# skitzoid/Box2D-MT

Measured on AMD Instinct MI355X. Metric: world steps/sec at 99858 bodies per GPU (BASELINE config 3: Tumbler 100k, CCD off; Step = collide + island solve + broad-phase + state read-back); for N > 1: container-steps/s = world steps/s x N containers in the one sharded world, higher is better.
Workload: dtype f32

## Files before the change

### box2d-mt_amd/csrc/b2d_kernels_collide.h

```cpp
#ifndef B2D_KERNELS_COLLIDE_H
#define B2D_KERNELS_COLLIDE_H

#include "b2d_world.h"
#include "b2d_toi.h"

__device__ __forceinline__ Xf loadXf(const float4* b_xf, int body)
{
	float4 t = b_xf[body];
	Xf xf;
	xf.p = v2(t.x, t.y);
	xf.q.s = t.z;
	xf.q.c = t.w;
	return xf;
}

__device__ __forceinline__ AABB loadAabb(const float4* p_fat, int proxy)
{
	float4 t = p_fat[proxy];
	AABB a;
	a.lo = v2(t.x, t.y);
	a.hi = v2(t.z, t.w);
	return a;
}

__device__ __forceinline__ bool bodyActiveForContact(uint32_t f)
{
	return (f & BF_AWAKE) != 0 && (f & BF_TYPE_MASK) != BT_STATIC;
}

__device__ __forceinline__ bool filterShouldCollide(uint32_t f0A, int f1A, uint32_t f0B, int f1B)
{
	int groupA = (int)(short)(f1A & 0xffff);
	int groupB = (int)(short)(f1B & 0xffff);
	if (groupA == groupB && groupA != 0)
	{
		return groupA > 0;
	}
	uint32_t catA = f0A & 0xffffu, maskA = f0A >> 16;
	uint32_t catB = f0B & 0xffffu, maskB = f0B >> 16;
	return (maskA & catB) != 0 && (catA & maskB) != 0;
}

__device__ __forceinline__ bool bodiesShouldCollide(const DW& W, int bodyA, int bodyB)
{
	uint32_t tA = W.b_flags[bodyA] & BF_TYPE_MASK;
	uint32_t tB = W.b_flags[bodyB] & BF_TYPE_MASK;
	if (tA != BT_DYNAMIC && tB != BT_DYNAMIC) return false;
	if (W.nJoints == 0) return true;
	for (int e = W.jadjStart[bodyA], end = W.jadjStart[bodyA + 1]; e < end; ++e)
	{
		const JointRec& jn = W.joints[W.jadj[e]];
		if (jn.bodyA == bodyB || jn.bodyB == bodyB)
		{
			if (jn.collideConnected == 0) return false;
		}
	}
	return true;
}

__device__ __forceinline__ bool isToiCandidate(const DW& W, int proxyA, int proxyB, int bodyA, int bodyB)
{
	const int fA = W.p_filter1[proxyA], fB = W.p_filter1[proxyB];
	if ((fA | fB) & PF_SENSOR) return false;
	const uint32_t bfA = W.b_flags[bodyA], bfB = W.b_flags[bodyB];
	if ((bfA | bfB) & BF_BULLET) return true;
	const bool includesNonDynamic = (bfA & BF_TYPE_MASK) != BT_DYNAMIC || (bfB & BF_TYPE_MASK) != BT_DYNAMIC;
	const bool neitherThick = ((fA | fB) & PF_THICK) == 0;
	return includesNonDynamic && neitherThick;
}

#define TOI_ORDER_SORT_MAX 2048
#define TOI_ORDER_SCRATCH_BYTES (TOI_ORDER_SORT_MAX * (8 + 4 * 4))
__device__ __forceinline__ void toiOrderDestroy(const DW& W, void* scratch)
{
	DState* S = W.st;
	const int n = __hip_atomic_load(&S->c.nToiDestroy, __ATOMIC_RELAXED, __HIP_MEMORY_SCOPE_AGENT);
	if (n == 0) return;
	const ContactArrays& C = W.ca[S->cur];
	uint64_t* s_key = (uint64_t*)scratch;
	int* s_sorted = (int*)(s_key + TOI_ORDER_SORT_MAX);
	int* s_slot = s_sorted + TOI_ORDER_SORT_MAX;
	int* s_tail = s_slot + TOI_ORDER_SORT_MAX;
	int* s_tailJ = s_tail + TOI_ORDER_SORT_MAX;
	const bool chunked = n > TOI_ORDER_SORT_MAX;
	uint64_t* g_key = W.pairKey;
	int* g_sorted = (int*)(W.pairKey + n);
	int* g_rank = W.toiList;
// ... 36 lines not shown
				for (int j = 0; j < m; ++j) rank += s_key[j] < key ? 1 : 0;
				const int ci = b2dLoadAgentI(&W.toiDestroyList[i]);
				s_sorted[rank] = ci;
				s_slot[rank] = C.mgr[ci];
			}
		}
		else
		{
			for (int i = threadIdx.x; i < m; i += blockDim.x)
			{
				const int ci = g_sorted[c0 + i];
				s_sorted[i] = ci;
				s_slot[i] = b2dLoadAgentI(&C.mgr[ci]);
			}
		}
		for (int t = threadIdx.x; t < count0 - base; t += blockDim.x) s_tail[t] = b2dLoadAgentI(&W.toiPos2c[base + t]);
		__syncthreads();
		for (int t = threadIdx.x; t < count0 - base; t += blockDim.x)
		{
			const int c = s_tail[t];
			int j = -1;
			if (b2dLoadAgentI((const int*)&C.flags[c]) & (int)CF_DESTROY)
			{
				if (!chunked) { for (int q = 0; q < m; ++q) if (s_sorted[q] == c) { j = q; break; } }
				else { const int r = g_rank[c]; if (r >= c0 && r < c0 + m) j = r - c0; }
			}
			s_tailJ[t] = j;
		}
		__syncthreads();
		if (threadIdx.x == 0)
		{
			for (int k = 0; k < m; ++k)
			{
				const int ci = s_sorted[k];
				const int slot = s_slot[k];
				--count;
				const int last = s_tail[count - base], lastJ = s_tailJ[count - base];
				W.toiPos2c[slot] = last;
				C.mgr[last] = slot;
				if (slot >= base) { s_tail[slot - base] = last; s_tailJ[slot - base] = lastJ; }
				if (lastJ >= 0) s_slot[lastJ] = slot;
				C.mgr[ci] = -1;
			}
			__threadfence();
		}
		count = count0 - m;
		__syncthreads();
	}
	if (threadIdx.x == 0)
	{
		S->c.nToiOrder = count;
		S->c.nToiDestroy = 0;
	}
}

__device__ __forceinline__ int collideClassKey(const DW& W, const ContactArrays& C, int i)
{
	const int4 ids = C.ids[i];
	const uint32_t flags = C.flags[i];
	if (flags & CF_FOREIGN) return 61;
	if (!(bodyActiveForContact(W.b_flags[ids.z]) || bodyActiveForContact(W.b_flags[ids.w]))) return 62;
	const float4 fA = W.p_fat[ids.x], fB = W.p_fat[ids.y];
	if (fB.x - fA.z > 0.0f || fB.y - fA.w > 0.0f || fA.x - fB.z > 0.0f || fA.y - fB.w > 0.0f) return 62;
	if (flags & CF_SENSOR) return 60;
	const ShapeRec* sA = W.shapes + W.p_shape[ids.x];
	const ShapeRec* sB = W.shapes + W.p_shape[ids.y];
	const int tA = sA->type == B2D_SHAPE_CHAIN ? B2D_SHAPE_EDGE : sA->type, tB = sB->type;
	const int cA = sA->count, cB = sB->count;
	auto bucket = [](int c) { return c < 3 ? 0 : (c > 8 ? 5 : c - 3); };
	if (tA == B2D_SHAPE_POLYGON && tB == B2D_SHAPE_POLYGON) return bucket(cA > cB ? cA : cB);
	if (tA == B2D_SHAPE_POLYGON && tB == B2D_SHAPE_CIRCLE) return 6 + bucket(cA);
	if (tA == B2D_SHAPE_CIRCLE && tB == B2D_SHAPE_CIRCLE) return 12;
	if (tA == B2D_SHAPE_EDGE && tB == B2D_SHAPE_POLYGON) return 13 + bucket(cB);
	if (tA == B2D_SHAPE_EDGE && tB == B2D_SHAPE_CIRCLE) return 19;
	return 59;
}

__device__ __forceinline__ bool b2dSameBits4(float4 a, float4 b)
{
	return __float_as_uint(a.x) == __float_as_uint(b.x) && __float_as_uint(a.y) == __float_as_uint(b.y) &&
		__float_as_uint(a.z) == __float_as_uint(b.z) && __float_as_uint(a.w) == __float_as_uint(b.w);
}

template <int STAGE, bool ORDER = true>
__global__ __launch_bounds__(256) void
__attribute__((amdgpu_waves_per_eu((!ORDER && !STAGE) ? 4 : 1, (!ORDER && !STAGE) ? 4 : 8)))
k_collide(DW W, int sortTile)
{
	b2dPhaseStamp(W);
	DState* S = W.st;
	const int n = S->c.nContacts;
	const ContactArrays& C = W.ca[S->cur];
	int nDestroy = 0, nTouch = 0;
	__shared__ int s_bin[64];
	__shared__ int s_perm[256];
	__shared__ __attribute__((aligned(16))) unsigned char s_raw[STAGE ? ((512 * sizeof(ShapeRec) > TOI_ORDER_SCRATCH_BYTES || !ORDER) ? 512 * sizeof(ShapeRec) : TOI_ORDER_SCRATCH_BYTES) : (ORDER ? TOI_ORDER_SCRATCH_BYTES : 16)];
	ShapeRec* const s_shape = (ShapeRec*)s_raw;
	__shared__ __attribute__((aligned(16))) ShapeRec s_uni[2];
	__shared__ int s_uniId[2];
	const bool uniOn = !STAGE && (sortTile & 4) != 0;
	sortTile &= 3;
	if (uniOn)
	{
		const int i0 = (int)(blockIdx.x * blockDim.x);
		int idA = 0, idB = 0;
		if (i0 < n)
		{
			const int4 ids0 = C.ids[i0];
			idA = W.p_shape[ids0.x];
			idB = W.p_shape[ids0.y];
		}
		static_assert(sizeof(ShapeRec) % 4 == 0, "ShapeRec is copied word by word");
		constexpr int RW = (int)(sizeof(ShapeRec) / 4);
		if (threadIdx.x < 2 * RW)
		{
			const int which = (int)threadIdx.x / RW, word = (int)threadIdx.x % RW;
			((uint32_t*)&s_uni[which])[word] = ((const uint32_t*)(W.shapes + (which ? idB : idA)))[word];
		}
		if (threadIdx.x == 0) { s_uniId[0] = idA; s_uniId[1] = idB; }
		__syncthreads();
	}
	for (int base = blockIdx.x * blockDim.x; base < n; base += gridDim.x * blockDim.x)
	{
		int i = base + (int)threadIdx.x;
		if (sortTile)
		{
			const int key = i < n ? collideClassKey(W, C, i) : 63;
			if (threadIdx.x < 64) s_bin[threadIdx.x] = 0;
			__syncthreads();
			const int within = atomicAdd(&s_bin[key], 1);
			__syncthreads();
			if (threadIdx.x < 64)
			{
				const int v = s_bin[threadIdx.x];
				int incl = v;
				for (int off = 1; off < 64; off <<= 1)
				{
					const int o = __shfl_up(incl, off);
					if ((int)threadIdx.x >= off) incl += o;
				}
				s_bin[threadIdx.x] = incl - v;
			}
			__syncthreads();
			s_perm[s_bin[key] + within] = (int)threadIdx.x;
			__syncthreads();
			i = base + s_perm[threadIdx.x];
		}
		if (i >= n) continue;
		int4 ids = C.ids[i];
		uint32_t flags = C.flags[i];
		if (flags & CF_FOREIGN)
		{
			int keepF = 1;
			if (flags & CF_FILTER)
			{
				const bool ok = bodiesShouldCollide(W, ids.w, ids.z) &&
					filterShouldCollide(W.p_filter0[ids.x], W.p_filter1[ids.x], W.p_filter0[ids.y], W.p_filter1[ids.y]);
				if (!ok) keepF = 0; else flags &= ~CF_FILTER;
			}
			if (keepF && (bodyActiveForContact(W.b_flags[ids.z]) || bodyActiveForContact(W.b_flags[ids.w])))
			{
				const float4 fA = W.p_fat[ids.x], fB = W.p_fat[ids.y];
				AABB boxA, boxB;
				boxA.lo = v2(fA.x, fA.y); boxA.hi = v2(fA.z, fA.w);
				boxB.lo = v2(fB.x, fB.y); boxB.hi = v2(fB.z, fB.w);
				if (!b2dAabbOverlap(boxA, boxB)) keepF = 0;
			}
			if (!keepF)
			{
				flags |= CF_DESTROY;
				++nDestroy;
				if (flags & CF_TOI_CANDIDATE) b2dStoreAgentI(&W.toiDestroyList[atomicAdd(&S->c.nToiDestroy, 1)], i);
			}
			C.flags[i] = flags;
			W.keepFlag[i] = keepF;
			continue;
		}
		const int4 m3 = C.man3[i];
		const float4 oldImp = C.imp[i];
		const float4 o0 = C.man0[i], o1 = C.man1[i];
		const int proxyA = ids.x, proxyB = ids.y, bodyA = ids.z, bodyB = ids.w;
		uint32_t bfA = W.b_flags[bodyA], bfB = W.b_flags[bodyB];
		const float4 fatA = W.p_fat[proxyA], fatB = W.p_fat[proxyB];
		const int shapeA = W.p_shape[proxyA], shapeB = W.p_shape[proxyB];
		const Xf xfA = loadXf(W.b_xf, bodyA), xfB = loadXf(W.b_xf, bodyB);
		int keep = 1;

		if (flags & CF_FILTER)
		{
			bool ok = bodiesShouldCollide(W, bodyB, bodyA) &&
				(W.userFilter ? (flags & CF_USER_REJECT) == 0
				              : filterShouldCollide(W.p_filter0[proxyA], W.p_filter1[proxyA], W.p_filter0[proxyB], W.p_filter1[proxyB]));
			flags &= ~CF_USER_REJECT;
			if (!ok)
			{
				keep = 0;
			}
			else
			{
				flags &= ~CF_FILTER;
			}
		}

		flags &= ~(CF_PRESOLVE | CF_VC_ONE_POINT);
		bool active = bodyActiveForContact(bfA) || bodyActiveForContact(bfB);
		if (keep && active)
		{
			AABB boxA, boxB;
			boxA.lo = v2(fatA.x, fatA.y); boxA.hi = v2(fatA.z, fatA.w);
			boxB.lo = v2(fatB.x, fatB.y); boxB.hi = v2(fatB.z, fatB.w);
			bool overlap = b2dAabbOverlap(boxA, boxB);
			if (!overlap)
			{
				keep = 0;
			}
			else if (flags & CF_FOREIGN)
			{
			}
			else
			{
				const uint32_t oldId0 = (uint32_t)m3.x, oldId1 = (uint32_t)m3.y;
				const int oldCount = m3.w;
				flags |= CF_ENABLED;
				bool wasTouching = (flags & CF_TOUCHING) != 0;
				bool touching = false;
				bool sensor = (flags & CF_SENSOR) != 0;
				float4 o0s = make_float4(0, 0, 0, 0), o1s = o0s;
				Manifold mf;
				mf.pointCount = 0;
				mf.type = m3.z;
				mf.id[0] = oldId0;
				mf.id[1] = oldId1;
				if (sensor)
				{
					const GjkProxy pA = b2dProxy(W.shapes + shapeA);
					const GjkProxy pB = b2dProxy(W.shapes + shapeB);
					GjkCache cache;
					cache.count = 0;
					cache.metric = 0.0f;
					for (int k = 0; k < 3; ++k) cache.indexA[k] = cache.indexB[k] = 0;
					GjkOutput dist;
					b2dDistance(dist, cache, pA, xfA, pB, xfB, true);
					touching = dist.distance < 10.0f * B2D_EPSILON;
					mf.pointCount = 0;
				}
				else
				{
					const ShapeRec* sA = W.shapes + shapeA;
					const ShapeRec* sB = W.shapes + shapeB;
					if (STAGE)
					{
						static_assert(sizeof(ShapeRec) % 8 == 0, "ShapeRec is copied in 8-byte pieces");
						const float2* gA = (const float2*)sA;
						const float2* gB = (const float2*)sB;
						float2* lA = (float2*)&s_shape[2 * threadIdx.x];
						float2* lB = (float2*)&s_shape[2 * threadIdx.x + 1];
#pragma unroll
						for (int q = 0; q < (int)(sizeof(ShapeRec) / 8); ++q) { lA[q] = gA[q]; lB[q] = gB[q]; }
						sA = &s_shape[2 * threadIdx.x];
						sB = &s_shape[2 * threadIdx.x + 1];
					}
					o0s = o0;
					o1s = o1;
					mf.localNormal = v2(o0.x, o0.y);
					mf.localPoint = v2(o0.z, o0.w);
					mf.p[0] = v2(o1.x, o1.y);
					mf.p[1] = v2(o1.z, o1.w);
					mf.id[0] = oldId0;
					mf.id[1] = oldId1;
					bool evaluated = false;
					if (uniOn)
					{
						const int u0 = s_uniId[0], u1 = s_uniId[1];
						const bool a0 = shapeA == u0, b0 = shapeB == u0;
						if ((a0 || shapeA == u1) && (b0 || shapeB == u1))
						{
							const ShapeRec* lA = &s_uni[a0 ? 0 : 1];
							const ShapeRec* lB = &s_uni[b0 ? 0 : 1];
							if (lA->type == B2D_SHAPE_POLYGON && lB->type == B2D_SHAPE_POLYGON && lA->count == 4 && lB->count == 4)
							{
								b2dCollidePolygons<4>(&mf, lA, xfA, lB, xfB);
								evaluated = true;
							}
						}
					}
					if (!evaluated) b2dEvaluate(&mf, sA, xfA, sB, xfB);
					touching = mf.pointCount > 0;
					float ni[2], ti[2];
					ni[0] = oldImp.x; ti[0] = oldImp.y; ni[1] = oldImp.z; ti[1] = oldImp.w;
					for (int k = 0; k < mf.pointCount; ++k)
					{
						mf.ni[k] = 0.0f;
						mf.ti[k] = 0.0f;
						uint32_t id2 = mf.id[k];
						if (oldCount > 0 && oldId0 == id2)
						{
							mf.ni[k] = oldImp.x;
							mf.ti[k] = oldImp.y;
						}
						else if (oldCount > 1 && oldId1 == id2)
						{
							mf.ni[k] = oldImp.z;
							mf.ti[k] = oldImp.w;
						}
						ni[k] = mf.ni[k];
						ti[k] = mf.ti[k];
					}
					if (touching != wasTouching)
					{
						W.b_wake[bodyA] = 1;
					}
					{
						const float4 n0 = make_float4(mf.localNormal.x, mf.localNormal.y, mf.localPoint.x, mf.localPoint.y);
						const float4 n1 = make_float4(mf.p[0].x, mf.p[0].y, mf.p[1].x, mf.p[1].y);
						const float4 nI = make_float4(ni[0], ti[0], ni[1], ti[1]);
						if (!b2dSameBits4(n0, o0)) C.man0[i] = n0;
						if (!b2dSameBits4(n1, o1)) C.man1[i] = n1;
						if (!b2dSameBits4(nI, oldImp)) C.imp[i] = nI;
					}
				}
				if (W.preSolveOn && !sensor && touching)
				{
					W.pre_o0[i] = o0s;
					W.pre_o1[i] = o1s;
					W.pre_oimp[i] = oldImp;
					W.pre_o3[i] = m3;
					flags |= CF_PRESOLVE;
				}
				{
					const int4 n3 = make_int4((int)mf.id[0], (int)mf.id[1], mf.type, mf.pointCount);
					if (n3.x != m3.x || n3.y != m3.y || n3.z != m3.z || n3.w != m3.w) C.man3[i] = n3;
				}
				if (touching) flags |= CF_TOUCHING; else flags &= ~CF_TOUCHING;
			}
		}

		if (!keep)
		{
			if (W.eventsOn && (flags & CF_REPORTED))
			{
				const int e = atomicAdd(&S->c.nEvents, 1);
				if (e < W.capContacts)
				{
					W.evKey[e] = C.key[i];
					W.evInfo[e] = make_int4(proxyA, proxyB, 1, -1);
				}
			}
			flags |= CF_DESTROY;
			++nDestroy;
			if (flags & CF_TOI_CANDIDATE) b2dStoreAgentI(&W.toiDestroyList[atomicAdd(&S->c.nToiDestroy, 1)], i);
			int pc = C.man3[i].w;
			if (pc > 0 && (flags & (CF_SENSOR | CF_FOREIGN)) == 0)
			{
				W.b_wake[bodyA] = 1;
				W.b_wake[bodyB] = 1;
			}
		}
		else if ((flags & (CF_TOUCHING | CF_FOREIGN)) == CF_TOUCHING)
		{
			++nTouch;
		}
		C.flags[i] = flags;
		W.keepFlag[i] = keep;
	}
	{
		__shared__ int s_census[2];
		if (threadIdx.x == 0) { s_census[0] = 0; s_census[1] = 0; }
		__syncthreads();
		nDestroy = waveSumInt(nDestroy);
		nTouch = waveSumInt(nTouch);
		if (waveLane() == 0)
		{
			if (nDestroy) atomicAdd(&s_census[0], nDestroy);
			if (nTouch) atomicAdd(&s_census[1], nTouch);
		}
		__syncthreads();
		const bool fit = (unsigned)W.capContacts <= TREE_SUM_MAX;
		if (!fit && threadIdx.x == 0)
		{
			if (s_census[0]) atomicAdd(&S->c.nDestroy, s_census[0]);
			if (s_census[1]) atomicAdd(&S->c.nTouching, s_census[1]);
		}
		unsigned t0 = 0u, t1 = 0u;
		if (b2dLastBlockArrive(W, ARRIVE_COLLIDE, fit ? (unsigned)s_census[0] : 0u, fit ? (unsigned)s_census[1] : 0u, &t0, &t1))
		{
			if (threadIdx.x == 0)
			{
				if (t0) atomicAdd(&S->c.nDestroy, (int)t0);
				if (t1) atomicAdd(&S->c.nTouching, (int)t1);
			}
			if (ORDER) toiOrderDestroy(W, s_raw);
		}
	}
}

__global__ __launch_bounds__(256) void k_toi_order_destroy(DW W)
{
	__shared__ __attribute__((aligned(16))) unsigned char s_raw[TOI_ORDER_SCRATCH_BYTES];
	toiOrderDestroy(W, s_raw);
}

__global__ __launch_bounds__(256) void k_contact_events(DW W)
{
	b2dPhaseStamp(W);
	DState* S = W.st;
	const int n = S->c.nContacts;
	const ContactArrays& C = W.ca[S->cur];
	for (int i = blockIdx.x * blockDim.x + threadIdx.x; i < n; i += gridDim.x * blockDim.x)
	{
		const uint32_t flags = C.flags[i];
		const bool touching = (flags & CF_TOUCHING) != 0, reported = (flags & CF_REPORTED) != 0;
		if (touching == reported || (flags & CF_FOREIGN) != 0) continue;
		C.flags[i] = flags ^ CF_REPORTED;
		const int e = atomicAdd(&S->c.nEvents, 1);
		if (e < W.capContacts)
		{
			const int4 ids = C.ids[i];
			W.evKey[e] = C.key[i];
			W.evInfo[e] = make_int4(ids.x, ids.y, touching ? 0 : 1, i);
		}
	}
}

__global__ __launch_bounds__(256) void k_presolve_gather(DW W)
{
	b2dPhaseStamp(W);
	DState* S = W.st;
	const int n = S->c.nContacts;
	const bool compacting = S->c.nDestroy != 0;
	const ContactArrays& C = W.ca[S->cur];
	for (int i = blockIdx.x * blockDim.x + threadIdx.x; i < n; i += gridDim.x * blockDim.x)
	{
		if (!W.keepFlag[i] || (C.flags[i] & CF_PRESOLVE) == 0) continue;
		C.flags[i] &= ~CF_PRESOLVE_OFF;
		const int e = atomicAdd(&S->c.nPreSolve, 1);
		if (e >= W.capContacts) continue;
		const int4 ids = C.ids[i];
		PreSolveRec r;
		r.info = make_int4(compacting ? W.keepScan[i] : i, ids.x, ids.y, 0);
		r.key = C.key[i];
		r.pad = 0ull;
		r.o0 = W.pre_o0[i]; r.o1 = W.pre_o1[i]; r.oimp = W.pre_oimp[i]; r.o3 = W.pre_o3[i];
		r.n0 = C.man0[i]; r.n1 = C.man1[i]; r.nimp = C.imp[i]; r.n3 = C.man3[i];
		r.mat = C.mat[i];
		W.preRecs[e] = r;
	}
}

__global__ __launch_bounds__(256) void k_presolve_disable(DW W, const int* list, int count)
{
	b2dPhaseStamp(W);
	const ContactArrays& C = W.ca[W.st->cur];
	for (int k = blockIdx.x * blockDim.x + threadIdx.x; k < count; k += gridDim.x * blockDim.x)
	{
		const int j = list[k];
		if (j >= 0 && j < W.st->c.nContacts) C.flags[j] = (C.flags[j] & ~CF_ENABLED) | CF_PRESOLVE_OFF;
	}
}

__global__ __launch_bounds__(256) void k_presolve_material(DW W, const int* list, int count)
{
	b2dPhaseStamp(W);
	const ContactArrays& C = W.ca[W.st->cur];
	for (int k = blockIdx.x * blockDim.x + threadIdx.x; k < count; k += gridDim.x * blockDim.x)
	{
		const int j = list[4 * k];
		if (j < 0 || j >= W.st->c.nContacts) continue;
		float4 m = C.mat[j];
		m.x = __int_as_float(list[4 * k + 1]);
		m.y = __int_as_float(list[4 * k + 2]);
		m.z = __int_as_float(list[4 * k + 3]);
		C.mat[j] = m;
	}
}

__global__ __launch_bounds__(256) void k_postsolve_gather(DW W)
// ... 47 lines not shown
	}
}

__global__ __launch_bounds__(256) void k_pairs_reject(DW W, const int* list, int count)
{
	b2dPhaseStamp(W);
	for (int k = blockIdx.x * blockDim.x + threadIdx.x; k < count; k += gridDim.x * blockDim.x) W.pairFirst[list[k]] = 0;
}

__global__ void k_step_begin(DW W, int* bar)
{
	b2dPhaseStamp(W);
	Counters& c = W.st->c;
	const int t = threadIdx.x;
	if (t == 0)
	{
		c.nDestroy = 0;
		(&c.nDestroy)[1] = 0;
		c.nPairs = 0;
		(&c.nPairs)[1] = 0;
		c.overflow = 0;
		c.cellExtBits = 0;
		c.gridFresh = 0;
		W.st->dbgCensus[0] = 0;
		c.nEvents = 0;
		c.nToiList = 0;
		c.nNewToiCand = 0;
		c.nToiEvents = 0;
		c.nToiCalls = 0;
		c.toiBase = 0;
		c.toiOverflow = 0;
		c.nToiLog = 0;
		c.toiIncomplete = 0;
		c.toiUnsafe = 0;
		c.nToiGroups = 0;
		c.nToiMoved = 0;
		c.nToiNewPairs = 0;
		c.nToiChainCreated = 0;
		c.nPreSolve = 0;
		c.nPostSolve = 0;
		c.nFilterList = 0;
		c.spToiCreated = 0;
		c.spToiStraddle = 0;
	}
	if (t < 32) bar[t] = t == 6 ? W.testSpinMax : 0;
	for (int k = t; k < ARRIVE_SITES * TREE_WORDS; k += (int)blockDim.x) W.arriveTree[k] = 0ull;
}

__global__ __launch_bounds__(256) void k_wake_apply(DW W)
{
	b2dPhaseStamp(W);
	for (int i = blockIdx.x * blockDim.x + threadIdx.x; i < W.nBodies; i += gridDim.x * blockDim.x)
	{
		if (W.b_wake[i])
		{
			W.b_flags[i] |= BF_AWAKE;
			W.b_pos[i].w = 0.0f;
			W.b_wake[i] = 0;
		}
	}
}

__global__ __launch_bounds__(256) void k_flag_filter(DW W, const unsigned long long* pairs, int nPairs)
{
	b2dPhaseStamp(W);
	DState* S = W.st;
	const int n = S->c.nContacts;
	const ContactArrays& C = W.ca[S->cur];
	for (int i = blockIdx.x * blockDim.x + threadIdx.x; i < n; i += gridDim.x * blockDim.x)
	{
		const int4 ids = C.ids[i];
		const unsigned lo = (unsigned)(ids.z < ids.w ? ids.z : ids.w), hi = (unsigned)(ids.z < ids.w ? ids.w : ids.z);
		const unsigned long long key = ((unsigned long long)lo << 32) | hi;
		int a = 0, b = nPairs;
		while (a < b)
		{
			const int m = (a + b) >> 1;
			if (pairs[m] < key) a = m + 1; else b = m;
		}
		if (a < nPairs && pairs[a] == key) C.flags[i] |= CF_FILTER;
	}
}

struct DW;
__device__ __forceinline__ bool keysetMaintained(const DW& W);
__device__ __forceinline__ bool htDelete(const DW& W, uint32_t mask, uint64_t key);

__global__ __launch_bounds__(256) void k_compact_contacts(DW W)
{
	b2dPhaseStamp(W);
	DState* S = W.st;
	if (S->c.nDestroy == 0) return;
	const int n = S->c.nContacts;
	const ContactArrays& A = W.ca[S->cur];
	const ContactArrays& B = W.ca[1 - S->cur];
	const bool ksOn = keysetMaintained(W);
	const uint32_t ksMask = S->c.ksMask;
	int ksTomb = 0, ksLost = 0;
	__shared__ int s_ks[2];
	if (threadIdx.x == 0) { s_ks[0] = 0; s_ks[1] = 0; }
	__syncthreads();
	for (int i = blockIdx.x * blockDim.x + threadIdx.x; i < n; i += gridDim.x * blockDim.x)
	{
		const int keep = W.keepFlag[i];
		const uint32_t fl = A.flags[i];
		const uint64_t key = A.key[i];
		if (!keep)
		{
			if (ksOn && (fl & CF_FOREIGN) == 0)
			{
				if (htDelete(W, ksMask, key + 1ull)) ksTomb += 1;
				else ksLost += 1;
			}
		}
		else
		{
			int j = W.keepScan[i];
			B.ids[j] = A.ids[i];
			B.key[j] = key;
			B.flags[j] = fl;
			if ((fl & CF_FOREIGN) == 0)
			{
				B.mat[j] = A.mat[i];
				B.man0[j] = A.man0[i];
				B.man1[j] = A.man1[i];
				B.imp[j] = A.imp[i];
				B.man3[j] = A.man3[i];
			}
			B.color[j] = A.color[i];
			const int m = A.mgr[i];
			B.mgr[j] = m;
			if (m >= 0) W.toiPos2c[m] = j;
		}
	}
	const bool fit = (unsigned)W.capContacts <= TREE_SUM_MAX;
	if (ksOn)
	{
		ksTomb = waveSumInt(ksTomb);
		ksLost = waveSumInt(ksLost);
		if (waveLane() == 0)
		{
			if (ksTomb) atomicAdd(&s_ks[0], ksTomb);
			if (ksLost) atomicAdd(&s_ks[1], ksLost);
		}
	}
	__syncthreads();
	unsigned tomb = (unsigned)s_ks[0], lost = (unsigned)s_ks[1];
	if (!fit && threadIdx.x == 0)
	{
		if (tomb) atomicAdd(&S->c.ksStats[KS_TOMBSTONES], (unsigned long long)tomb);
		if (lost) { atomicAdd(&S->c.ksStats[KS_NOT_FOUND], (unsigned long long)lost); S->c.ksStale = 1; }
	}
	if (b2dLastBlockArrive(W, ARRIVE_COMPACT, fit ? tomb : 0u, fit ? lost : 0u, &tomb, &lost) && threadIdx.x == 0)
	{
		if (fit && tomb) S->c.ksStats[KS_TOMBSTONES] += (unsigned long long)tomb;
		if (fit && lost) { S->c.ksStats[KS_NOT_FOUND] += (unsigned long long)lost; S->c.ksStale = 1; }
		S->c.nContacts = W.keepScan[n];
		S->cur = 1 - S->cur;
	}
}

#define HT_TOMB 0xffffffffffffffffull

__device__ __forceinline__ uint32_t hashKey(uint64_t k)
{
	k ^= k >> 33;
	k *= 0xff51afd7ed558ccdULL;
	k ^= k >> 33;
	k *= 0xc4ceb9fe1a85ec53ULL;
	k ^= k >> 33;
// ... 99 lines not shown
```

### box2d-mt_amd/csrc/b2hip_api_callbacks.h

```cpp

int b2hip_set_contact_filter(b2hip_world* w, b2hip_should_collide_fn fn, void* user)
{
	if (int rcu = checkUsable(w, "b2hip_set_contact_filter", true)) return rcu;
	w->filterFn = fn;
	w->filterUser = user;
	w->dw.userFilter = hasFilter(w) ? 1 : 0;
	return B2HIP_OK;
}

int b2hip_set_contact_filter_batch(b2hip_world* w, b2hip_should_collide_batch_fn fn, void* user)
{
	if (int rcu = checkUsable(w, "b2hip_set_contact_filter_batch", true)) return rcu;
	w->filterBatchFn = fn;
	if (fn) w->filterUser = user;
	w->dw.userFilter = hasFilter(w) ? 1 : 0;
	return B2HIP_OK;
}

int b2hip_default_should_collide(b2hip_world* w, int fixture_a, int fixture_b)
{
	if (!w || fixture_a < 0 || fixture_b < 0 || fixture_a >= (int)w->fixtures.size() || fixture_b >= (int)w->fixtures.size())
		return setError(B2HIP_ERR_INVALID, "bad fixture id");
	const HostFixture& a = w->fixtures[fixture_a];
	const HostFixture& b = w->fixtures[fixture_b];
// ... 121 lines not shown
		std::vector<uint32_t> f(nb);
		if (nb && hipMemcpy(f.data(), w->b_flags.p, nb * 4, hipMemcpyDeviceToHost) != hipSuccess) bad = 1;
		for (size_t i = 0; i < nb; ++i) f[i] &= 0x7fu;
		h = fnv(h, f.data(), nb * 4);
	}
	else if (which == 1)
	{
		bad |= pull(w->c_ids[cur].p, nc * 16); bad |= pull(w->c_key[cur].p, nc * 8);
		std::vector<uint32_t> f(nc);
		if (nc && hipMemcpy(f.data(), w->c_flags[cur].p, nc * 4, hipMemcpyDeviceToHost) != hipSuccess) bad = 1;
		for (size_t i = 0; i < nc; ++i) f[i] &= 0x1fu;
		h = fnv(h, f.data(), nc * 4);
		bad |= pull(w->c_man0[cur].p, nc * 16); bad |= pull(w->c_man1[cur].p, nc * 16);
		bad |= pull(w->c_imp[cur].p, nc * 16); bad |= pull(w->c_man3[cur].p, nc * 16);
	}
	else if (which == 2)
	{
		bad |= pull(w->p_fat.p, np * 16);
	}
	else
	{
		bad |= pull(w->c_imp[cur].p, nc * 16);
	}
	if (bad) return setError(B2HIP_ERR_HIP, "debug hash read-back failed");
	*out = h;
	return 0;
}

int b2hip_debug_read(b2hip_world* w, int which, int first, int count, void* out)
{
	if (!w) return setError(B2HIP_ERR_INVALID, "null world");
	DEVICE_GUARD(w);
	if (!w || !out) return setError(B2HIP_ERR_INVALID, "null argument");
	HIP_TRY(hipStreamSynchronize(w->stream));
	const void* src = nullptr;
	size_t elem = 16;
	switch (which)
	{
	case 0: src = w->b_pos.p; break;
	case 1: src = w->b_vel.p; break;
	case 2: src = w->li_bodies.p; elem = 4; break;
	case 3: src = w->b_force.p; break;
	case 4: src = w->b_flags.p; elem = 4; break;
	case 5: src = w->b_damp.p; break;
	case 6: src = w->b_mass.p; break;
	case 7: src = w->d_state.p; elem = 4; break;
	case 8: src = w->dbgPreVel.p; break;
	case 9: src = w->dbgVel.p; break;
	case 10: src = w->dbgLi.p; elem = 4; break;
	case 11: src = w->gridBar.p; elem = 4; break;
	case 12:
	{
		if (first < 0 || count < 0 || first + count > COLOR_SLOT_PADDED) return setError(B2HIP_ERR_INVALID, "colour census: [0, 65)");
		HIP_TRY(hipStreamSynchronize(w->stream));
		if (count > 0) HIP_TRY(hipMemcpy2D(out, sizeof(int), w->colorCount.p + colorSlot(first), COLOR_SLOT_STRIDE * sizeof(int), sizeof(int), (size_t)count, hipMemcpyDeviceToHost));
		return 0;
	}
	case 13: src = w->bodyColorMask.p; elem = 8; break;
	case 14: src = w->deg.p; elem = 4; break;
	case 15: src = w->hubList.p; elem = 4; break;
	case 16: src = w->bodyActive.p; elem = 8; break;
	case 17: src = w->b_blk1.p; elem = 4; break;
	case 18: src = w->li_ref.p; break;
	case 19: src = w->rowColor.p; elem = 4; break;
	case 20: src = w->blkRowStart.p; elem = 4; break;
	case 21: src = w->bodyRest.p; elem = 8; break;
	case 22:
	{
		const long long stats[2] = { w->statSorts, w->statSortsOnepass };
		if (first < 0 || count < 0 || first + count > 2) return setError(B2HIP_ERR_INVALID, "pair-update statistics: [0, 2)");
		memcpy(out, stats + first, (size_t)count * sizeof(long long));
		return 0;
	}
	case 23:
	{
		if (first < 0 || count < 0 || first + count > KS_STATS + 2) return setError(B2HIP_ERR_INVALID, "key-set statistics: [0, 12)");
		Counters c;
		HIP_TRY(hipMemcpy(&c, &w->d_state.p->c, sizeof(Counters), hipMemcpyDeviceToHost));
		long long stats[KS_STATS + 2];
		for (int k = 0; k < KS_STATS; ++k) stats[k] = (long long)c.ksStats[k];
		stats[KS_STATS] = c.ksFill;
		stats[KS_STATS + 1] = c.ksMask;
		memcpy(out, stats + first, (size_t)count * sizeof(long long));
		return 0;
	}
	default: return setError(B2HIP_ERR_INVALID, "bad array id");
	}
	HIP_TRY(hipMemcpy(out, (const char*)src + (size_t)first * elem, (size_t)count * elem, hipMemcpyDeviceToHost));
	return 0;
}

int b2hip_test_radix_sort(b2hip_world* w, int count, uint64_t* keys, int* payloads, int passes, const int* shifts, const int* widths)
{
	if (!w) return setError(B2HIP_ERR_INVALID, "null world");
	DEVICE_GUARD(w);
	if (count < 0 || passes < 1 || !shifts || !widths || (count > 0 && (!keys || !payloads))) return setError(B2HIP_ERR_INVALID, "bad argument");
	if (w->stepActive) return setError(B2HIP_ERR_INVALID, "inside a step");
	std::vector<std::pair<int, int>> lay;
	for (int p = 0; p < passes; ++p)
	{
		if (widths[p] < 1 || widths[p] > RADIX_BITS || shifts[p] < 0 || shifts[p] + widths[p] > 64) return setError(B2HIP_ERR_INVALID, "bad pass");
		lay.push_back(std::make_pair(shifts[p], widths[p]));
	}
	int rc = ensureCapacity(w, 0);
	if (rc) return rc;
	hipStream_t s = w->stream;
	const int tilesCap = count / RADIX_TILE + 1;
	const size_t tiles = (size_t)tilesCap + 1;
	rc = w->radixHist.ensure(RADIX_DIGITS * tiles + 2, s); if (rc) return rc;
	rc = w->radixHistScan.ensure(RADIX_DIGITS * tiles + 4, s); if (rc) return rc;
	rc = w->scanTmp.ensure(3 * (RADIX_DIGITS * tiles / SCAN_TILE + 8), s); if (rc) return rc;
	rc = w->scanFlags.ensure(RADIX_DIGITS * tiles / SCAN_TILE + 8, s); if (rc) return rc;
	if (w->sortOnepass)
	{
		const size_t onepassTiles = std::min<size_t>(tiles, RADIX_ONEPASS_MAX_TILES);
		rc = w->radixCounts.ensure(onepassTiles * RADIX_DIGITS, s, false); if (rc) return rc;
		rc = w->radixGroups.ensure((onepassTiles / RADIX_GROUP + 1) * RADIX_DIGITS, s, false); if (rc) return rc;
	}
	rc = ensureCapacity(w, 0);
	if (rc) return rc;
	DevArray<uint64_t> k0, k1;
	DevArray<int2> v0, v1;
	DevArray<int> nDev;
	const size_t room = (size_t)count + 1;
	rc = k0.ensure(room, s, false, false);
	if (!rc) rc = k1.ensure(room, s, false, false);
	if (!rc) rc = v0.ensure(room, s, false, false);
	if (!rc) rc = v1.ensure(room, s, false, false);
	if (!rc) rc = nDev.ensure(1, s, false, true);
	auto done = [&](int code) { (void)hipStreamSynchronize(s); k0.release(); k1.release(); v0.release(); v1.release(); nDev.release(); return code; };
	if (rc) return done(rc);
	hipError_t e = hipMemcpyAsync(nDev.p, &count, sizeof(int), hipMemcpyHostToDevice, s);
	if (e == hipSuccess && count > 0) e = hipMemcpyAsync(k0.p, keys, (size_t)count * sizeof(uint64_t), hipMemcpyHostToDevice, s);
	if (e == hipSuccess && count > 0) e = hipMemcpyAsync(v0.p, payloads, (size_t)count * sizeof(int2), hipMemcpyHostToDevice, s);
	if (e != hipSuccess) return done(setError(B2HIP_ERR_HIP, hipGetErrorString(e)));
	uint64_t *kin = k0.p, *kout = k1.p;
	int2 *vin = v0.p, *vout = v1.p;
	rc = radixSort(w, kin, kout, vin, vout, nDev.p, tilesCap, lay);
	if (rc) return done(rc);
	int overflow = 0;
	e = hipMemcpyAsync(&overflow, &w->d_state.p->c.overflow, sizeof(int), hipMemcpyDeviceToHost, s);
	if (e == hipSuccess && count > 0) e = hipMemcpyAsync(keys, kin, (size_t)count * sizeof(uint64_t), hipMemcpyDeviceToHost, s);
	if (e == hipSuccess && count > 0) e = hipMemcpyAsync(payloads, vin, (size_t)count * sizeof(int2), hipMemcpyDeviceToHost, s);
	if (e == hipSuccess) e = hipStreamSynchronize(s);
	if (e != hipSuccess) return done(setError(B2HIP_ERR_HIP, hipGetErrorString(e)));
	if (overflow & SCAN_ABORT_BIT) return done(setError(B2HIP_ERR_HIP, "a look-back of the sort gave up waiting for a predecessor tile"));
	return done(0);
}

__global__ __launch_bounds__(256) void k_keyset_check(DW W, unsigned long long* out)
{
	const DState* S = W.st;
	const ContactArrays& C = W.ca[S->cur];
	const uint32_t mask = S->c.ksMask;
	const int stride = (int)(gridDim.x * blockDim.x), t0 = (int)(blockIdx.x * blockDim.x + threadIdx.x);
	int missing = 0, own = 0, live = 0, tomb = 0;
	for (int i = t0; i < S->c.nContacts; i += stride)
	{
		if (C.flags[i] & CF_FOREIGN) continue;
		own += 1;
		const uint64_t key = C.key[i] + 1ull;
		uint32_t h = hashKey(key) & mask;
		bool found = false;
		for (uint32_t probes = 0; probes <= mask; ++probes)
		{
			const uint64_t v = W.ht_keys[h];
// ... 172 lines not shown
```

### box2d-mt_amd/csrc/b2hip_api_snapshot.h

```cpp

namespace
{
struct SnapHeader
{
	char magic[8];
	uint32_t version, szDState, szHostBody, szHostFixture, szShape, szJoint;
	uint32_t nBodies, nFixtures, nShapes, nJoints, nFree, nContacts, nToiOrder, nMoves;
	uint32_t stateCount, cur;
	int32_t nextNode, leafCount, lastContacts, newFixture;
	float inv_dt0, cellSize;
	int32_t eventsOn, solverHints;
};
const uint32_t kSnapVersion = 6;
const char kSnapMagic[8] = { 'B', '2', 'H', 'I', 'P', 'S', 'N', '1' };

struct SnapWriter
{
	std::vector<char> out;
	void host(const void* p, size_t n) { const char* c = (const char*)p; out.insert(out.end(), c, c + n); }
	int dev(const void* p, size_t n)
	{
		const size_t at = out.size();
		out.resize(at + n);
		if (n == 0) return 0;
// ... 197 lines not shown
	{
		uint32_t tail[2];
		in.host(tail, sizeof(tail));
		if (tail[1] != sizeof(GearRec) || tail[0] > size) return corrupt("gear section");
		nG = tail[0];
		gearsAt = (const GearRec*)in.take(nG * sizeof(GearRec));
		if (!gearsAt && nG) return setError(B2HIP_ERR_INVALID, "snapshot truncated");
	}
	for (size_t k = 0; k < nJ; ++k)
	{
		RevoluteJoint j;
		memcpy((void*)&j, jointsAt + k, sizeof(j));
		if (j.type < B2D_JOINT_DEAD || j.type > B2D_JOINT_GEAR) return corrupt("joint type");
		if (j.bodyA < 0 || (size_t)j.bodyA >= nb || j.bodyB < 0 || (size_t)j.bodyB >= nb) return corrupt("joint bodies");
		if (j.type == B2D_JOINT_GEAR && (j.enableLimit < 0 || (size_t)j.enableLimit >= nG)) return corrupt("gear index");
	}
	for (size_t k = 0; k < nG; ++k)
	{
		GearRec g;
		memcpy((void*)&g, gearsAt + k, sizeof(g));
		if (g.bodyC < 0 || (size_t)g.bodyC >= nb || g.bodyD < 0 || (size_t)g.bodyD >= nb) return corrupt("gear bodies");
	}

	def.device = device;
	b2hip_world* w = nullptr;
	int rc = b2hip_world_create(&def, &w);
	if (rc) return rc;
	DEVICE_GUARD(w);
	auto fail = [&](int code) { const std::string why = g_lastError; b2hip_world_destroy(w); return setError(code, why); };
	w->bodies.resize(nb);
	for (size_t i = 0; i < nb; ++i)
	{
		memcpy((void*)&w->bodies[i], bodiesAt + i * bodyBytes, offsetof(HostBody, fixtures));
		w->bodies[i].dirty = bodiesAt[i * bodyBytes + offsetof(HostBody, fixtures)] != 0;
		w->bodies[i].pullEpoch = 0;
		w->bodies[i].forceEpoch = w->stepEpoch;
		if (w->bodies[i].dirty) w->dirtyList.push_back((int)i);
	}
	{
		size_t count = 0;
		for (size_t i = 0; i < nb; ++i) count += w->bodies[i].worldIndex >= 0 ? 1 : 0;
		w->nonStatic.assign(count, -1);
		for (size_t i = 0; i < nb; ++i)
		{
			const int k = w->bodies[i].worldIndex;
			if (k < 0) continue;
			if ((size_t)k >= count || w->nonStatic[(size_t)k] != -1) return fail(corrupt("non-static body order"));
			w->nonStatic[(size_t)k] = (int)i;
		}
		w->orderDirty = true;
	}
	w->fixtures.resize(np);
	if (np) memcpy(w->fixtures.data(), fixturesAt, np * sizeof(HostFixture));
	w->shapes.resize(nS);
	if (nS) memcpy((void*)w->shapes.data(), shapesAt, nS * sizeof(ShapeRec));
	w->freeUnits.resize(h.nFree);
	if (h.nFree) memcpy(w->freeUnits.data(), freeAt, (size_t)h.nFree * sizeof(FreeUnit));
	for (size_t f = 0; f < np; ++f) w->bodies[w->fixtures[f].body].fixtures.push_back((int)f);
	for (size_t k = 0; k < nS; ++k) w->shapeIndex[std::string((const char*)&w->shapes[k], sizeof(ShapeRec))] = (int)k;
	w->joints.resize(nJ);
	if (nJ) memcpy((void*)w->joints.data(), jointsAt, nJ * sizeof(RevoluteJoint));
	for (size_t k = 0; k < nJ; ++k) w->nMouseJoints += w->joints[k].type == B2D_JOINT_MOUSE;
	w->gears.resize(nG);
	if (nG) memcpy((void*)w->gears.data(), gearsAt, nG * sizeof(GearRec));
	w->nextNode = h.nextNode; w->leafCount = h.leafCount; w->lastContacts = h.lastContacts; w->newFixture = h.newFixture != 0;
	w->inv_dt0 = h.inv_dt0;
	w->eventsOn = h.eventsOn != 0;
	w->serialOrphansNext = h.solverHints & 1;
	w->blocksTooBig = (h.solverHints & 2) != 0;
	w->stepComplete = (h.solverHints & 4) == 0;
	w->adoptSticky = (h.solverHints >> 8) & 0xff;
	w->largeHintSteps = (h.solverHints >> 16) & 0xff;
	w->recolorCountdown = (h.solverHints >> 24) & 0x7f;
	w->freshColors = ((h.solverHints >> 3) & 0x1f) | ((int)(((uint32_t)h.solverHints >> 31) & 1u) << 5);
	w->freshColorsPending = false;
	w->adoptPasses = w->adoptSticky > 0;
	rc = ensureCapacity(w, nC);
	if (rc) return fail(rc);
	if (nM > w->moveBuf.cap || nC > (size_t)w->dw.capContacts || (size_t)h.stateCount * 10 > w->h_stateCap) return fail(corrupt("counts exceed the buffers sized for them"));
	if (h.stateCount) memcpy(w->h_state, stateAt, (size_t)h.stateCount * 10 * sizeof(float));
	w->shadowDev = nullptr;
	w->stateCount = h.stateCount;
	*w->h_dstate = ds;
#define SNAP_UP(arr, s) do { if ((s).bytes && hipMemcpy(w->arr.p, (s).p, (s).bytes, hipMemcpyHostToDevice) != hipSuccess) return fail(setError(B2HIP_ERR_HIP, "snapshot upload failed (" #arr ")")); } while (0)
	if (hipMemcpy(w->d_state.p, &ds, sizeof(DState), hipMemcpyHostToDevice) != hipSuccess) return fail(setError(B2HIP_ERR_HIP, "snapshot upload failed (state block)"));
	w->pubSeq = ds.pubCount;
	SNAP_UP(b_pos, sPos); SNAP_UP(b_pos0, sPos0); SNAP_UP(b_vel, sVel); SNAP_UP(b_xf, sXf); SNAP_UP(b_mass, sMass); SNAP_UP(b_damp, sDamp);
	w->forceOnDevice = true; w->rowsWentEarly = false;
	SNAP_UP(b_force, sForce); SNAP_UP(b_flags, sFlags); SNAP_UP(b_wake, sWake); SNAP_UP(b_proxyHead, sHead); SNAP_UP(b_blk1, sBlk);
	SNAP_UP(p_fat, sFat); SNAP_UP(p_body, sPBody); SNAP_UP(p_shape, sPShape); SNAP_UP(p_key, sPKey); SNAP_UP(p_filter0, sF0); SNAP_UP(p_filter1, sF1);
	SNAP_UP(p_mat, sPMat); SNAP_UP(p_next, sNext);
	const int cur = (int)h.cur;
	SNAP_UP(c_ids[cur], cIds); SNAP_UP(c_key[cur], cKey); SNAP_UP(c_flags[cur], cFlags); SNAP_UP(c_mat[cur], cMat); SNAP_UP(c_man0[cur], cMan0);
	SNAP_UP(c_man1[cur], cMan1); SNAP_UP(c_imp[cur], cImp); SNAP_UP(c_man3[cur], cMan3); SNAP_UP(c_color[cur], cColor); SNAP_UP(c_mgr[cur], cMgr);
	SNAP_UP(toiPos2c, sToi); SNAP_UP(moveBuf, sMoves);
#undef SNAP_UP
	if (nS && hipMemcpy(w->d_shapes.p, w->shapes.data(), nS * sizeof(ShapeRec), hipMemcpyHostToDevice) != hipSuccess)
		return fail(setError(B2HIP_ERR_HIP, "snapshot upload failed (shapes)"));
	w->upBodies = nb; w->upFixtures = np; w->upShapes = nS; w->upJoints = 0;
	w->dw.cellSize = h.cellSize;
	w->dw.invCellSize = 1.0f / h.cellSize;
	w->dw.eventsOn = w->eventsOn ? 1 : 0;
	*out = w;
	return B2HIP_OK;
}

int b2hip_get_contacts(b2hip_world* w, int cap, b2hip_contact* out)
{
	if (!w) return setError(B2HIP_ERR_INVALID, "null world");
	DEVICE_GUARD(w);
	if (!w || !out) return setError(B2HIP_ERR_INVALID, "null argument");
	int rc = flushForRead(w);
	if (rc) return rc;
	rc = readState(w);
	if (rc) return rc;
	const int n = std::min(cap, w->h_dstate->c.nContacts);
	const int cur = w->h_dstate->cur;
	if (n <= 0) return 0;
	std::vector<int4> ids(n), m3(n);
	std::vector<uint32_t> flags(n);
	std::vector<float4> mat(n), m0(n), m1(n), imp(n);
	HIP_TRY(hipMemcpy(ids.data(), w->c_ids[cur].p, n * sizeof(int4), hipMemcpyDeviceToHost));
	HIP_TRY(hipMemcpy(m3.data(), w->c_man3[cur].p, n * sizeof(int4), hipMemcpyDeviceToHost));
	HIP_TRY(hipMemcpy(flags.data(), w->c_flags[cur].p, n * sizeof(uint32_t), hipMemcpyDeviceToHost));
	HIP_TRY(hipMemcpy(mat.data(), w->c_mat[cur].p, n * sizeof(float4), hipMemcpyDeviceToHost));
	HIP_TRY(hipMemcpy(m0.data(), w->c_man0[cur].p, n * sizeof(float4), hipMemcpyDeviceToHost));
	HIP_TRY(hipMemcpy(m1.data(), w->c_man1[cur].p, n * sizeof(float4), hipMemcpyDeviceToHost));
	HIP_TRY(hipMemcpy(imp.data(), w->c_imp[cur].p, n * sizeof(float4), hipMemcpyDeviceToHost));
	for (int i = 0; i < n; ++i)
	{
		b2hip_contact& c = out[i];
		c.fixture_a = ids[i].x;
		c.fixture_b = ids[i].y;
		c.body_a = ids[i].z;
		c.body_b = ids[i].w;
		c.flags = ((flags[i] & CF_TOUCHING) ? 1u : 0u) | ((flags[i] & CF_ENABLED) ? 2u : 0u);
		c.manifold_type = m3[i].z;
		c.point_count = m3[i].w;
		c.local_normal[0] = m0[i].x; c.local_normal[1] = m0[i].y;
		c.local_point[0] = m0[i].z; c.local_point[1] = m0[i].w;
		c.point_local[0][0] = m1[i].x; c.point_local[0][1] = m1[i].y;
		c.point_local[1][0] = m1[i].z; c.point_local[1][1] = m1[i].w;
		c.normal_impulse[0] = imp[i].x; c.tangent_impulse[0] = imp[i].y;
		c.normal_impulse[1] = imp[i].z; c.tangent_impulse[1] = imp[i].w;
		c.id_key[0] = (uint32_t)m3[i].x;
		c.id_key[1] = (uint32_t)m3[i].y;
		c.friction = mat[i].x;
		c.restitution = mat[i].y;
		c.tangent_speed = mat[i].z;
	}
	return n;
}
```

### box2d-mt_amd/csrc/b2hip_api_step.h

```cpp

int b2hip_step_begin(b2hip_world* w, float dt, int velocity_iterations, int position_iterations)
{
	if (int rc = checkUsable(w, "b2hip_step_begin", false)) return rc;
	if (w->stepActive) return setError(B2HIP_ERR_INVALID, "b2hip_step_begin inside a step (finish it with b2hip_step_end)");
	DEVICE_GUARD(w);
	return stepFailed(w, stepBeginImpl(w, dt, velocity_iterations, position_iterations));
}

static bool keyLess(const std::pair<unsigned long long, int>& a, const std::pair<unsigned long long, int>& b) { return a < b; }

static void toManifold(b2hip_manifold* m, float4 m0, float4 m1, float4 imp, int4 m3)
{
	m->type = m3.z;
	m->point_count = m3.w;
	m->local_normal[0] = m0.x; m->local_normal[1] = m0.y;
	m->local_point[0] = m0.z; m->local_point[1] = m0.w;
	m->point_local[0][0] = m1.x; m->point_local[0][1] = m1.y;
	m->point_local[1][0] = m1.z; m->point_local[1][1] = m1.w;
	m->normal_impulse[0] = imp.x; m->tangent_impulse[0] = imp.y;
	m->normal_impulse[1] = imp.z; m->tangent_impulse[1] = imp.w;
	m->id_key[0] = (uint32_t)m3.x;
	m->id_key[1] = (uint32_t)m3.y;
}

// ... 557 lines not shown
		}
	}
	w->events.clear();
	if (w->h_dstate->c.rowsSkipped == 1)
	{
		rc = downloadState(w, -1);
		if (rc) return rc;
	}
	if (w->eventsOn)
	{
		LAUNCH(w, k_contact_events, gridFor(w->dw.capContacts), 256, w->dw);
		int nEv = 0;
		HIP_TRY(hipMemcpyAsync(&nEv, &w->d_state.p->c.nEvents, sizeof(int), hipMemcpyDeviceToHost, w->stream));
		HIP_TRY(hipStreamSynchronize(w->stream));
		if (nEv > w->dw.capContacts) return setError(B2HIP_ERR_CAPACITY, "contact event buffer overflow");
		if (nEv > 0)
		{
			std::vector<unsigned long long> keys(nEv);
			std::vector<int4> info(nEv);
			HIP_TRY(hipMemcpy(keys.data(), w->evKey.p, nEv * sizeof(unsigned long long), hipMemcpyDeviceToHost));
			HIP_TRY(hipMemcpy(info.data(), w->evInfo.p, nEv * sizeof(int4), hipMemcpyDeviceToHost));
			std::vector<int> order(nEv);
			for (int i = 0; i < nEv; ++i) order[i] = i;
			std::sort(order.begin(), order.end(), [&](int a, int b)
			{
				if (info[a].z != info[b].z) return info[a].z < info[b].z;
				return keys[a] < keys[b];
			});
			w->events.resize(nEv);
			for (int i = 0; i < nEv; ++i)
			{
				const int4 q = info[order[i]];
				w->events[i].fixture_a = q.x;
				w->events[i].fixture_b = q.y;
				w->events[i].kind = q.z;
				w->events[i].contact_index = q.w;
			}
		}
	}
	if (w->debugSync) HIP_TRY(hipStreamSynchronize(w->stream));
	refreshMirror(w);
	const Counters& c = w->h_dstate->c;
	w->lastContacts = c.nContacts;
	w->last.nContacts = c.nContacts;
	w->last.nMoves = c.nMoves;
	if (c.nMovesSeen > 256 && !w->gridForced)
	{
		long long rounds = 0;
		for (int k = 0; k < 32; ++k) rounds += c.candRounds[k];
		const double perProxy = 64.0 * (double)rounds / (double)c.nMovesSeen;
		if (perProxy > 128.0) w->gridHalf = true; else if (perProxy < 48.0) w->gridHalf = false;
		w->dw.gridHalf = w->gridHalf ? 1 : 0;
	}
	w->last.nNewContacts = c.nNewContacts;
	w->last.nPairs = c.nPairs;
	w->last.overflow = c.overflow;
	if (w->colorSmallPending)
	{
		w->colorSmallPending = false;
		w->last.nColors = c.nColors;
		if (c.overflow & 4) return setError(B2HIP_ERR_CAPACITY, "more than 64 constraint colours on one body");
		if (c.nUncolored != 0) return setError(B2HIP_ERR_CAPACITY, "incremental colouring did not converge");
	}
	if ((c.overflow & 0x2040) == 0x2040) return setError(B2HIP_ERR_CAPACITY, "a block of the large-island partition holds more rows or home bodies than its workgroup takes (the census the host partitions by did not see them)");
	if (c.overflow & 64)
	{
		if (w->handoverWhy) handoverPostMortem(w);
		return setError(B2HIP_ERR_HIP, "a wait inside a resident large-island solver timed out (a workgroup was not resident, or a hand-over never came)");
	}
	if (c.overflow & SCAN_ABORT_BIT) return setError(B2HIP_ERR_HIP, "a single-pass scan gave up waiting for a predecessor tile (k_scan_chain look-back)");
	w->last.posItersLarge = c.posItersLarge;
	w->last.nHubRows = c.nHubRows;
	w->last.hubRounds = c.hubRounds;
	w->last.hubSerialChunks = c.hubSerialChunks;
	w->toiChainContacts += c.nToiChainCreated;
	if (w->toiRan)
	{
		w->last.toiUnsafe = c.toiUnsafe;
		w->last.nToiEvents = c.nToiEvents;
		w->last.nToiCalls = c.nToiCalls;
		w->last.toiOverflow = c.toiOverflow;
		if (c.toiOverflow) return setError(B2HIP_ERR_CAPACITY, "TOI event scratch overflow (flags " + std::to_string(c.toiOverflow) + ")");
	}
	if (w->sp.dt > 0.0f) w->inv_dt0 = w->sp.inv_dt;
	if (w->def.continuous && w->sp.dt > 0.0f) w->stepComplete = c.toiIncomplete == 0;
	w->stepActive = false;

	float ms = 0.0f;
	float* p = w->profile;
	memset(p, 0, sizeof(float) * 13);
	{
		const unsigned long long* pc0 = w->h_dstate->phaseClock;
		p[0] = pc0[13] > pc0[14] ? 1.0e-5f * (float)(pc0[13] - pc0[14]) : 0.0f;
	}
	if (w->profileDetail)
	{
	const unsigned long long* pc = w->h_dstate->phaseClock;
	auto span = [pc](int a, int b) -> float { return pc[b] > pc[a] ? 1.0e-5f * (float)(pc[b] - pc[a]) : 0.0f; };
	p[1] = span(1, 2);
	p[2] = span(2, 3);
	p[3] = span(2, 4);
	const float dfs = span(4, 5), small = span(5, 6), color = span(6, 7), large = span(7, 8);
	p[3] += dfs + color;
	p[5] = small + large;
	const float bpTop = span(0, 1), bp0 = span(3, 9), bp1 = span(9, 10);
	p[10] = bp0;
	p[11] = bp1 + bpTop;
	p[9] = bp0 + bp1 + bpTop;
	if (w->toiEventValid) p[7] = span(10, 12);
	w->solverMs = small + large;
	if (w->blocksThisStep && w->h_dstate->stamps[4] > 0)
	{
		const float tick = 1.0e-5f;
		const float total = tick * (float)w->h_dstate->stamps[4];
		const float scale = total > 0.0f ? large / total : 0.0f;
		p[4] = scale * tick * (float)w->h_dstate->stamps[0];
		p[5] = small + scale * tick * (float)(w->h_dstate->stamps[2] - w->h_dstate->stamps[0]);
		p[6] = scale * tick * (float)(w->h_dstate->stamps[4] - w->h_dstate->stamps[2]);
	}
	}
	const int Ct = w->last.nSContacts + w->last.nLContacts;
	const int B = w->last.nSBodies + w->last.nLBodies;
	w->solverConstraints = Ct;
	w->solverBodies = B;
	w->solverBytes = (double)Ct * (w->sp.velIters * 220.0 + w->sp.posIters * 136.0 + 488.0) + (double)B * 240.0;
	w->ktMs = 0.0f;
	w->ktLaunches = 0;
	w->ktBytes = 0.0;
	if (w->kernelTiming && w->ktUsed >= 2)
	{
		for (int k = 0; k + 1 < w->ktUsed; k += 2)
		{
			float t = 0.0f;
			(void)hipEventElapsedTime(&t, w->ktEvents[k], w->ktEvents[k + 1]);
			w->ktMs += t;
			w->ktLaunches += 1;
		}
		if (w->ktKind == 5) w->ktBytes = (double)w->ktUnitsA * 480.0 + (double)w->ktUnitsB * 230.0;
		else if (w->ktKind == 6) w->ktBytes = (double)w->ktUnitsA * 250.0;
		else if (w->ktKind == 7) w->ktBytes = (double)w->ktUnitsA * 16.0 + (double)w->ktUnitsB * 8.0;
		else if (w->ktKind == 1) w->ktBytes = (double)w->last.nLContacts * 220.0 * w->sp.velIters;
		else if (w->ktKind == 8)
		{
			w->ktBytes = (double)w->last.nLContacts * (w->sp.velIters * 220.0 + w->last.posItersLarge * 136.0 + 488.0) + (double)w->last.nLBodies * 240.0;
			w->ktLaunches = w->familyLaunches;
		}
		else if (w->ktKind == 4) w->ktBytes = (double)w->last.nLContacts * (w->sp.velIters * 220.0 + w->last.posItersLarge * 136.0 + 488.0) + (double)w->last.nLBodies * 240.0;
		else w->ktBytes = (double)w->last.nSContacts * (w->sp.velIters * 220.0 + w->sp.posIters * 136.0 + 488.0) + (double)w->last.nSBodies * 240.0;
	}
	return 0;
}

int b2hip_set_lazy_readback(b2hip_world* w, int enable)
{
	if (int rc = checkUsable(w, "b2hip_set_lazy_readback", true)) return rc;
	ensureRows(w);
	w->lazyReadback = enable != 0;
	return w->failed ? setError(B2HIP_ERR_HIP, w->failedWhy) : B2HIP_OK;
}

int b2hip_step_end(b2hip_world* w)
{
	if (int rc = checkUsable(w, "b2hip_step_end", false)) return rc;
	if (!w->stepActive) return setError(B2HIP_ERR_INVALID, "b2hip_step_end outside a step");
	DEVICE_GUARD(w);
	const int rc = stepFailed(w, stepEndImpl(w));
// ... 88 lines not shown
```

### box2d-mt_amd/csrc/b2hip_api_world.h

```cpp


const char* b2hip_last_error(void)
{
	return g_lastError.c_str();
}

const char* b2hip_version(void)
{
	return "b2hip 0.1 (gfx950)";
}

int b2hip_world_create(const b2hip_world_def* def, b2hip_world** out)
{
	if (!def || !out) return setError(B2HIP_ERR_INVALID, "null argument");
	int count = 0;
	hipError_t e = hipGetDeviceCount(&count);
	if (e != hipSuccess || count <= 0)
	{
		return setError(B2HIP_ERR_NO_DEVICE, "no HIP device available: the b2hip Step() path has no CPU fallback");
	}
	int current = 0;
	if (hipGetDevice(&current) != hipSuccess) current = 0;
	const int device = def->device >= 0 ? def->device : current;
	if (device >= count) return setError(B2HIP_ERR_NO_DEVICE, "no such HIP device");
// ... 102 lines not shown
		return setError(B2HIP_ERR_HIP, "hipHostMalloc failed");
	}
	if (hipHostMalloc((void**)&w->h_pub, sizeof(DState), hipHostMallocMapped | hipHostMallocCoherent) != hipSuccess ||
		hipHostGetDevicePointer((void**)&w->d_pub, w->h_pub, 0) != hipSuccess)
	{
		b2hip_world_destroy(w);
		return setError(B2HIP_ERR_HIP, "hipHostMalloc (coherent) failed");
	}
	memset(w->h_pub, 0, sizeof(DState));
	if (hipHostMalloc((void**)&w->h_pub2, sizeof(DState), hipHostMallocMapped | hipHostMallocCoherent) != hipSuccess ||
		hipHostGetDevicePointer((void**)&w->d_pub2, w->h_pub2, 0) != hipSuccess)
	{
		b2hip_world_destroy(w);
		return setError(B2HIP_ERR_HIP, "hipHostMalloc (coherent) failed");
	}
	memset(w->h_pub2, 0, sizeof(DState));
	if (hipHostMalloc((void**)&w->h_solverWord, 64, hipHostMallocMapped | hipHostMallocCoherent) != hipSuccess ||
		hipHostGetDevicePointer((void**)&w->d_solverWord, w->h_solverWord, 0) != hipSuccess)
	{
		b2hip_world_destroy(w);
		return setError(B2HIP_ERR_HIP, "hipHostMalloc (coherent) failed");
	}
	memset(w->h_solverWord, 0, 64);
	int rc = ensureCapacity(w, 0);
	if (rc == 0 && hipStreamSynchronize(w->stream) != hipSuccess) rc = setError(B2HIP_ERR_HIP, "stream sync failed");
	if (rc)
	{
		const std::string why = g_lastError;
		b2hip_world_destroy(w);
		return setError(rc, why);
	}
	*out = w;
	return B2HIP_OK;
}

void b2hip_world_destroy(b2hip_world* w)
{
	if (!w) return;
	DEVICE_GUARD(w);
	if (w->stream) (void)hipStreamSynchronize(w->stream);
	if (w->rowStream)
	{
		(void)hipStreamSynchronize(w->rowStream);
		(void)hipStreamDestroy(w->rowStream);
		(void)hipEventDestroy(w->rowFork);
		(void)hipEventDestroy(w->rowJoin);
		w->rowStream = nullptr;
	}
	if (w->shardComm != nullptr && g_rcclDestroy != nullptr) g_rcclDestroy(w->shardComm);
	w->shardComm = nullptr;
	w->shardSend.release(); w->shardRecv.release();
	w->b_owner.release(); w->spNewOwner.release(); w->spAwake.release(); w->spStraddle.release(); w->spCount.release(); w->spTarget.release();
	w->spSend.release(); w->spRecv.release(); w->spTailKey.release(); w->spVirt.release();
	if (w->spHost) (void)hipHostFree(w->spHost);
	w->spHost = nullptr;
	if (w->spOwnHost) (void)hipHostFree(w->spOwnHost);
	w->spOwnHost = nullptr;
	if (w->spHdrHost) (void)hipHostFree(w->spHdrHost);
	w->spHdrHost = nullptr;
	for (size_t k = 0; k < w->spTape.size(); ++k) (void)hipFree(w->spTape[k].first);
	w->spTape.clear();
	w->d_state.release();
	w->b_pos.release(); w->b_pos0.release(); w->b_vel.release(); w->b_xf.release(); w->b_mass.release(); w->b_damp.release();
	w->b_force.release(); w->b_flags.release(); w->b_wake.release(); w->b_rowDirty.release();
	w->p_fat.release(); w->p_body.release(); w->p_shape.release(); w->p_key.release(); w->p_filter0.release(); w->p_filter1.release();
	w->p_mat.release(); w->d_shapes.release();
	for (int k = 0; k < 2; ++k)
	{
		w->c_ids[k].release(); w->c_key[k].release(); w->c_flags[k].release(); w->c_mat[k].release(); w->c_man0[k].release();
		w->c_man1[k].release(); w->c_imp[k].release(); w->c_man3[k].release(); w->c_color[k].release();
	}
	w->ht_keys.release(); w->d_joints.release(); w->d_gears.release(); w->li_ref.release();
	w->jadjStart.release(); w->jadj.release(); w->rootJointStart.release(); w->rootJointCursor.release();
	w->lj_list.release(); w->rootJointOkay.release();
	w->parent.release(); w->rootSeed.release(); w->rootBodies.release(); w->rootContacts.release(); w->rootJoints.release();
	w->rootIsland.release(); w->deg.release(); w->adjStart.release(); w->adjCursor.release(); w->adj.release(); w->adjSlot.release();
	w->rootScanIn.release(); w->rootScanOut.release();
	w->si_root.release(); w->si_bodyStart.release(); w->si_contactStart.release(); w->si_wStart.release(); w->si_maxLevel.release();
	w->si_bodies.release(); w->si_contacts.release(); w->si_level.release(); w->si_stack.release(); w->si_lastLevel.release();
	w->b_slot.release(); w->b_island.release(); w->chunkFirst.release();
	w->li_bodies.release(); w->li_contacts.release(); w->li_roots.release(); w->li_color.release(); w->colorCount.release();
	w->colorStart.release(); w->colorCursor.release(); w->li_sorted.release(); w->bodyClaim.release(); w->rootPen.release();
	w->bodyActive.release(); w->bodyRest.release(); w->b_posv.release(); w->evKey.release(); w->evInfo.release(); w->uncolList.release(); w->compactList.release(); w->gridBar.release(); w->hubRowOf.release(); w->hubList.release(); w->hubDelta.release(); w->hubMeta.release(); w->hubFirst.release(); w->solveSnapBody.release(); w->solveSnapImp.release(); w->solveSnapCFlags.release(); w->solveSnapJoints.release(); w->solveSnapGears.release();
	w->b_proxyHead.release(); w->p_next.release(); w->toiList.release(); w->toiPos2c.release(); w->toiDestroyList.release(); w->toiNewList.release();
	w->b_toiGroup.release(); w->toiGroups.release(); w->toiGroupCount.release(); w->toiGroupList.release(); w->toiMoved.release(); w->toiNew.release(); w->toiParent.release(); w->toiDomOf.release(); w->toiDomRoot.release(); w->toiDomCount.release(); w->toiDomBase.release(); w->toiDomFill.release(); w->toiDomFailed.release(); w->toiDomEvents.release(); w->toiDomList.release(); w->toiHull.release(); w->snapBody.release(); w->snapFat.release();
	w->c_mgr[0].release(); w->c_mgr[1].release(); w->dbgPreVel.release(); w->dbgVel.release(); w->dbgLi.release();
	w->rootSleepMin.release(); w->bodyColorMask.release(); w->rootDone.release(); w->lc.release(); w->warmDelta.release();
	w->moveBuf.release(); w->gridCount.release(); w->gridStart.release(); w->gridCursor.release(); w->gridItems.release(); w->gridFat.release(); w->arriveTree.release();
	w->largeProxies.release(); w->largeMoves.release(); w->pairKey.release(); w->pairKey2.release(); w->pairProxy.release(); w->pairProxy2.release();
	w->filterPairs.release();
	w->d_editOps.release();
	w->b_order.release(); w->orderBody.release(); w->bigRoots.release();
	w->pre_o0.release(); w->pre_o1.release(); w->pre_oimp.release(); w->pre_o3.release(); w->preRecs.release();
	w->postRecs.release(); w->filterList.release(); w->hostList.release(); w->toiLog.release(); w->toiVerdict.release();
	w->b_blk1.release(); w->b_adopt.release(); w->b_adoptStage.release(); w->blkRows.release(); w->blkRowStart.release(); w->blkCursor.release(); w->blkBodyCount.release(); w->blkBodyCursor.release();
	w->blkBodyStart.release(); w->blkBodies.release(); w->rowColor.release(); w->b_cutv.release();
	w->pairFirst.release(); w->pairRank.release(); w->scanTmp.release(); w->radixHist.release(); w->radixHistScan.release();
	w->keepFlag.release(); w->keepScan.release(); w->scanTmp4.release(); w->scanFlags.release(); w->radixCounts.release(); w->radixGroups.release(); w->radixGlobalHist.release(); w->stateOut.release(); w->consts.release();
	w->qIn.release(); w->qCounts.release(); w->qOffsets.release(); w->qItems.release(); w->qFlags.release(); w->qScanWork.release();
	w->qScanWords.release(); w->qWords.release(); w->qHits.release(); w->qDistances.release(); w->qPoses.release(); w->qShapes.release();
	w->qKeys.release(); w->qKeysWork.release(); w->qAny.release();
	if (w->qPinned) (void)hipHostFree(w->qPinned);
	if (w->h_state) (void)hipHostFree(w->h_state);
	if (w->h_dstate) (void)hipHostFree(w->h_dstate);
	if (w->h_pub) (void)hipHostFree(w->h_pub);
	if (w->h_pub2) (void)hipHostFree(w->h_pub2);
	if (w->h_solverWord) (void)hipHostFree(w->h_solverWord);
	for (int i = 0; i < 13; ++i)
		if (w->ev[i]) (void)hipEventDestroy(w->ev[i]);
	for (size_t i = 0; i < w->ktEvents.size(); ++i) (void)hipEventDestroy(w->ktEvents[i]);
	if (w->stream) (void)hipStreamDestroy(w->stream);
	if (w->stream2) (void)hipStreamDestroy(w->stream2);
	if (w->evFork) (void)hipEventDestroy(w->evFork);
	if (w->evJoin) (void)hipEventDestroy(w->evJoin);
	delete w;
}

int b2hip_set_gravity(b2hip_world* w, float gx, float gy)
{
	if (int rcu = checkUsable(w, "b2hip_set_gravity", true)) return rcu;
	if (!w) return setError(B2HIP_ERR_INVALID, "null world");
	w->def.gravity_x = gx;
	w->def.gravity_y = gy;
	return 0;
}

int b2hip_set_flags(b2hip_world* w, int allow_sleep, int warm_starting, int continuous, int sub_stepping)
{
	if (int rcu = checkUsable(w, "b2hip_set_flags", true)) return rcu;
	if (!w) return setError(B2HIP_ERR_INVALID, "null world");
	w->def.allow_sleep = allow_sleep;
	w->def.warm_starting = warm_starting;
	w->def.continuous = continuous;
	w->def.sub_stepping = sub_stepping;
	return 0;
}

int b2hip_create_body(b2hip_world* w, const b2hip_body_def* def)
{
	if (!w || !def) return setError(B2HIP_ERR_INVALID, "null argument");
	if (int rcu = checkUsable(w, "b2hip_create_body", true)) return rcu;
	HostBody b{};
	b.type = def->type;
	b.flags = 0;
	if (def->bullet) b.flags |= BF_BULLET;
	if (def->fixed_rotation) b.flags |= BF_FIXEDROT;
	if (def->allow_sleep) b.flags |= BF_AUTOSLEEP;
	if (def->awake) b.flags |= BF_AWAKE;
	if (def->active) b.flags |= BF_ACTIVE;
	b.px = def->px;
	b.py = def->py;
	b.qs = sinf(def->angle);
	b.qc = cosf(def->angle);
	b.lcx = b.lcy = 0.0f;
	b.c0x = b.cx = def->px;
	b.c0y = b.cy = def->py;
	b.a0 = b.a = def->angle;
	b.vx = def->vx;
	b.vy = def->vy;
	b.w = def->w;
	b.linearDamping = def->linear_damping;
	b.angularDamping = def->angular_damping;
	b.gravityScale = def->gravity_scale;
	b.fx = b.fy = b.torque = 0.0f;
	b.sleepTime = 0.0f;
	b.pullEpoch = w->mirrorEpoch;
	b.forceEpoch = w->stepEpoch;
// ... 1121 lines not shown
```

### box2d-mt_amd/csrc/b2hip_host_phases.h

```cpp

static int spExchangeState(b2hip_world* w, int mode);
static int spExchangePairs(b2hip_world* w, long long* totalPairs, int* straddling);
static int spResolve(b2hip_world* w, int nVirt = 0);
static int spAfterToi(b2hip_world* w);
static int spBeginStep(b2hip_world* w);

static int radixBits(int maxKey)
{
	int bits = 1;
	while ((1 << bits) <= maxKey && bits < 31) ++bits;
	return bits;
}

static void radixPasses(int first, int bits, std::vector<std::pair<int, int>>& out)
{
	const int passes = (bits + RADIX_BITS - 1) / RADIX_BITS;
	for (int p = 0, at = 0; p < passes; ++p)
	{
		const int width = (bits - at + (passes - p) - 1) / (passes - p);
		out.push_back(std::make_pair(first + at, width));
		at += width;
	}
}

// ... 66 lines not shown

static int userFilterPairs(b2hip_world* w, const int2* proxies)
{
	int rc = readState(w);
	if (rc) return rc;
	const int n = std::min(w->h_dstate->c.nPairs, w->dw.capPairs);
	if (n <= 0 || (w->h_dstate->c.overflow & 3)) return 0;
	std::vector<int> first(n);
	std::vector<int2> pr(n);
	HIP_TRY(hipMemcpy(first.data(), w->pairFirst.p, (size_t)n * sizeof(int), hipMemcpyDeviceToHost));
	HIP_TRY(hipMemcpy(pr.data(), proxies, (size_t)n * sizeof(int2), hipMemcpyDeviceToHost));
	std::vector<int> refused, asked, which, verdict;
	for (int i = 0; i < n; ++i)
	{
		if (!first[i]) continue;
		asked.push_back(pr[i].x);
		asked.push_back(pr[i].y);
		which.push_back(i);
	}
	askFilter(w, asked, verdict);
	for (size_t k = 0; k < which.size(); ++k) if (!verdict[k]) refused.push_back(which[k]);
	return applyHostList(w, k_pairs_reject, refused);
}

static int runSortAndCreate(b2hip_world* w, bool largePath, long long knownPairs = -1)
{
	DW& d = w->dw;
	const uint64_t* sortedKeys = d.pairKey;
	const int2* sortedProxies = d.pairProxy;
	if (largePath)
	{
		int bits = radixBits(w->nextNode + 1);
		std::vector<std::pair<int, int>> passes;
		radixPasses(0, bits, passes);
		radixPasses(32, bits, passes);
		uint64_t* kin = d.pairKey;
		uint64_t* kout = d.pairKey2;
		int2* vin = d.pairProxy;
		int2* vout = d.pairProxy2;
		int tilesCap = d.capPairs / RADIX_TILE + 1;
		if (knownPairs >= 0) tilesCap = (int)std::min<long long>(tilesCap, knownPairs / RADIX_TILE + 2);
		if (int rcs = radixSort(w, kin, kout, vin, vout, &d.st->c.nPairs, tilesCap, passes)) return rcs;
		sortedKeys = kin;
		sortedProxies = vin;
		LAUNCH(w, k_pairs_sorted_first, gridFor(d.capPairs), 256, d, sortedKeys, w->consts.p + 3);
		if (hasFilter(w)) { int rcf = userFilterPairs(w, sortedProxies); if (rcf) return rcf; }
		deviceExclusiveScan<int>(w->stream, d.pairFirst, d.pairRank, d.scanTmp, w->scanCtx, w->consts.p + 3,
			knownPairs >= 0 ? (int)std::min<long long>(d.capPairs, knownPairs + 2) : d.capPairs);
		LAUNCH(w, k_pairs_sorted_total, 1, 1, d, w->consts.p + 3);
	}
	else
	{
		LAUNCH(w, k_pairs_first, 16, 256, d);
		if (hasFilter(w)) { int rcf = userFilterPairs(w, sortedProxies); if (rcf) return rcf; }
		LAUNCH(w, k_pairs_rank, 16, 256, d);
	}
	const int smallPath = largePath ? 0 : 1;
	LAUNCH(w, k_create_contacts, gridFor(largePath ? d.capPairs : COUNT_RANK_MAX), 256, d, sortedKeys, sortedProxies, smallPath);
	LAUNCH(w, k_create_finish, gridFor(d.nBodies), 256, d, smallPath);
	LAUNCH(w, k_toi_order_create, 1, 1024, d, smallPath);
	return 0;
}

static int findNewContacts(b2hip_world* w, bool sync);
static int findNewContactsOnce(b2hip_world* w, bool sync);
static int findNewContactsGraph(b2hip_world* w)
{
	if (hasFilter(w) || w->spatial) return findNewContacts(w, true);
	return findNewContacts(w, w->pairsLargeSticky > 0);
}

static int growPairBuffers(b2hip_world* w)
{
	const Counters& c = w->h_dstate->c;
	if (c.overflow & 2) w->pairCapHint = 2 * (size_t)c.nPairs + 4096;
	int rc = ensureCapacity(w, (size_t)c.nContacts + (size_t)std::max(c.nNewContacts, 0) + 1024);
	if (rc) return rc;
	HIP_TRY(hipMemsetAsync(&w->d_state.p->c.overflow, 0, sizeof(int), w->stream));
	return 0;
}

static int findNewContacts(b2hip_world* w, bool sync)
{
	for (int attempt = 0; sync && attempt < 4; ++attempt)
	{
		int rc = findNewContactsOnce(w, true);
		if (rc != 1) return rc;
	}
	if (sync) return setError(B2HIP_ERR_CAPACITY, "pair buffer overflow");
	return findNewContactsOnce(w, false);
}

static int findNewContactsOnce(b2hip_world* w, bool sync)
{
	DW& d = w->dw;
	LAUNCH(w, k_bp_clear, gridFor(std::max(d.htMask, d.gridMask) + 1), 256, d);
	LAUNCH(w, k_bp_build, gridFor(std::max(d.capContacts, d.nProxies)), 256, d);
	deviceExclusiveScan<int>(w->stream, d.gridCount, d.gridStart, d.scanTmp, w->scanCtx, w->consts.p + 1, (int)(d.gridMask + 1));
	LAUNCH(w, k_grid_fill, gridFor(d.nProxies), 256, d, 0);
	if (int rk = ktBracket(w, 4, 7)) return rk;
	if (d.gridHalf) LAUNCH(w, k_find_pairs_window, gridFor((size_t)d.capMoves * 64, 256, 2048), 256, d);
	else LAUNCH(w, k_find_pairs_small, gridFor((size_t)d.capMoves * 64, 256, 2048), 256, d);
	if (int rk = ktBracket(w, 4, 7)) return rk;
	LAUNCH(w, k_find_pairs_large, 1024, 256, d);
	bool large = false;
	if (w->spatial)
	{
		long long total = 0;
		int straddle = 0;
		int rc = spExchangePairs(w, &total, &straddle);
		if (rc) return rc;
		large = total > COUNT_RANK_MAX;
		rc = runSortAndCreate(w, large, total);
		if (rc) return rc;
		if (straddle == 0)
		{
			HIP_TRY(hipMemsetAsync(&w->d_state.p->c.nStraddle, 0, 4 * sizeof(int), w->stream));
			LAUNCH(w, k_sp_flag_contacts, gridFor(d.capContacts), 256, d);
			return 0;
		}
		return spResolve(w);
	}
	if (sync)
	{
		int rc = startEarlyRows(w);
		if (rc) return rc;
		rc = readState(w);
		if (rc) return rc;
		if (w->h_dstate->c.overflow & 3)
		{
			rc = growPairBuffers(w);
			return rc ? rc : 1;
		}
		if (w->h_dstate->c.nMoves == 0) { if (w->pairsLargeSticky > 0) w->pairsLargeSticky -= 1; return 0; }
		large = w->h_dstate->c.nPairs > COUNT_RANK_MAX;
		if (large) w->pairsLargeSticky = 16;
		else if (w->pairsLargeSticky > 0) w->pairsLargeSticky -= 1;
	}
	return runSortAndCreate(w, large, sync ? (long long)w->h_dstate->c.nPairs : -1);
}

static int phaseCollide(b2hip_world* w)
{
	const bool split = w->collideSplitEnv < 0 ? w->last.nContacts >= 262144 : w->collideSplitEnv != 0;
	DW& d = w->dw;
	if (int rk = ktBracket(w, 2, 5)) return rk;
	const bool many = w->shapes.size() > 4096;
	const bool stage = w->collideStage < 0 ? many : w->collideStage != 0;
	const int sort = w->collideSortEnv < 0 ? (many ? 1 : 0) : (w->collideSortEnv != 0 ? 1 : 0);
	const int uni = w->collideUniOff ? 0 : 4;
	if (stage) LAUNCH(w, (k_collide<1, true>), gridFor(d.capContacts), 256, d, sort);
	else if (split)
	{
		LAUNCH(w, (k_collide<0, false>), gridFor(d.capContacts), 256, d, sort | uni);
		LAUNCH(w, k_toi_order_destroy, 1, 256, d);
	}
	else LAUNCH(w, (k_collide<0, true>), gridFor(d.capContacts), 256, d, sort | uni);
	if (int rk = ktBracket(w, 2, 5)) return rk;
	deviceExclusiveScan<int>(w->stream, d.keepFlag, d.keepScan, d.scanTmp, w->scanCtx, &d.st->c.nContacts, d.capContacts);
	if (d.preSolveOn) LAUNCH(w, k_presolve_gather, gridFor(d.capContacts), 256, d);
	LAUNCH(w, k_compact_contacts, gridFor(d.capContacts), 256, d);
	return 0;
}

int b2hip_debug_hash(b2hip_world* w, int which, uint64_t* out);
static void tracePoint(b2hip_world* w, const char* label)
{
	if (!w->debugTrace) return;
	uint64_t hb = 0, hi = 0;
	(void)b2hip_debug_hash(w, 0, &hb);
	(void)b2hip_debug_hash(w, 3, &hi);
	w->trace.push_back(std::make_pair(std::string(label), hb ^ (hi * 0x9E3779B97F4A7C15ull)));
}
#define TRACE(label) tracePoint(w, label)

static int partitionLargeIslands(b2hip_world* w, int targetDeg)
{
	DW& d = w->dw;
	HIP_TRY(hipMemcpyAsync(&w->d_state.p->c.blkTargetDeg, &targetDeg, sizeof(int), hipMemcpyHostToDevice, w->stream));
	uint64_t* kin = d.pairKey;
	uint64_t* kout = d.pairKey2;
	int2* vin = d.pairProxy;
	int2* vout = d.pairProxy2;
	LAUNCH(w, k_part_keys, gridFor(d.nBodies), 256, d, kin, vin);
	std::vector<std::pair<int, int>> passes;
	const int idBits = radixBits(d.nBodies + 1);
	radixPasses(0, idBits, passes);
	radixPasses(32, 32, passes);
	const int tilesCap = std::min(d.capPairs / RADIX_TILE + 1, d.nBodies / RADIX_TILE + 2);
	const int* nPtr = &d.st->c.nLBodies;
	if (int rcs = radixSort(w, kin, kout, vin, vout, nPtr, tilesCap, passes)) return rcs;
	LAUNCH(w, k_part_weights, gridFor(d.nBodies), 256, d, vin, d.pairFirst);
	deviceExclusiveScan<int>(w->stream, d.pairFirst, d.pairRank, d.scanTmp, w->scanCtx, nPtr, d.nBodies);
	LAUNCH(w, k_part_assign, gridFor(d.nBodies), 256, d, vin, d.pairRank);
	LAUNCH(w, k_color_recheck_begin, gridFor(d.nBodies), 256, d);
	LAUNCH(w, k_color_check, gridFor(d.capContacts), 256, d);
	LAUNCH(w, k_color_masks, gridFor(d.nBodies), 256, d);
	LAUNCH(w, k_block_census, 1, 1024, d, (DState*)nullptr);
	return 0;
}

struct SolveStep
{
	Counters c;
	bool poll = false;
	bool largeHint = false;
	bool exactLarge = false;
	bool colorSmallQueued = false;
	bool colorAheadPublished = false;
	bool plainIslands = false;
	bool blockShape = false;
	bool hasJoints = false, hasHubs = false;
	bool sideStream = false;
	bool smallDeferred = false;
	int nLIslands = 0, nLBodies = 0, nLContacts = 0, nColors = 0;
	bool useBlocks = false;
	bool useSweep = false;
	bool colorsOnDevice = false;
	bool censusVoid = false;
	bool colorSpill = false;
};

static const int RECOLOR_SLACK = 2;

static int buildIslands(b2hip_world* w, const SolveStep& s)
{
	DW& d = w->dw;
	const bool adopt = w->adoptPasses;
	const int pubBy = !s.poll ? 0 : (s.largeHint ? 1 : ((d.nJoints == 0 && !adopt) ? 2 : 3));
	int solidRounds = 1;
	while (solidRounds < SOLID_TILE_ROUNDS_MAX && (long long)w->last.nContacts >= 2ll * solidRounds * 256 * 1024) solidRounds *= 2;
	if (w->solidRoundsEnv > 0) solidRounds = w->solidRoundsEnv;
	const int gSolid = gridFor((size_t)(d.capContacts + solidRounds - 1) / solidRounds);
// ... 1184 lines not shown
```

### box2d-mt_amd/csrc/b2hip_host_world.h

```cpp

static thread_local std::string g_lastError;

static int setError(int code, const std::string& msg)
{
	g_lastError = msg;
	return code;
}

#define HIP_TRY(expr)                                                                                   \
	do                                                                                                  \
	{                                                                                                   \
		hipError_t _e = (expr);                                                                         \
		if (_e != hipSuccess)                                                                           \
		{                                                                                               \
			return setError(B2HIP_ERR_HIP, std::string(#expr) + ": " + hipGetErrorString(_e));          \
		}                                                                                               \
	} while (0)

static void (*g_rcclDestroy)(void* comm) = nullptr;

template <typename T>
struct DevArray
{
	T* p = nullptr;
// ... 141 lines not shown
	DevArray<int4> evInfo;
	bool eventsOn = false;
	std::vector<b2hip_contact_event> events;
	std::vector<b2hip_toi_callback> toiCallbacks;
	DevArray<ToiLogRec> toiLog;
	DevArray<int4> toiVerdict;
	DevArray<int> uncolList, compactList, hubRowOf, hubList;
	DevArray<float4> hubDelta, warmDelta;
	DevArray<unsigned long long> hubMeta, hubFirst;
	DevArray<int> rootDone;
	DevArray<float> lc;
	DevArray<int> moveBuf, gridCount, gridStart, gridCursor, gridItems, largeProxies, largeMoves;
	DevArray<float4> gridFat;
	DevArray<unsigned long long> arriveTree;
	DevArray<uint64_t> pairKey, pairKey2;
	DevArray<int2> pairProxy, pairProxy2;
	DevArray<int> pairFirst, pairRank;
	DevArray<int> scanTmp, radixHist, radixHistScan, keepFlag, keepScan;
	DevArray<int4> scanTmp4;
	DevArray<float4> qIn;
	DevArray<int> qCounts, qOffsets, qItems, qFlags, qScanWork, qScanWords, qWords;
	DevArray<b2hip_ray_hit> qHits;
	DevArray<b2hip_distance_hit> qDistances;
	DevArray<unsigned long long> qKeys, qKeysWork;
	DevArray<uint8_t> qAny;
	DevArray<QueryPose> qPoses;
	DevArray<ShapeRec> qShapes;
	ScanFlags qScan;
	void* qPinned = nullptr;
	size_t qPinnedBytes = 0;
	void* shardComm = nullptr;
	DevArray<int> shardSend, shardRecv;
	size_t shardExchangeBytes = 0;
	bool shardLoopback = false;
	bool spatial = false;
	DevArray<uint8_t> b_owner, spNewOwner, spAwake;
	bool spFullRows = false;
	int spRowCap = 1024, spProxyCap = 4096;
	int spIdle[6] = {0, 0, 0, 0, 0, 0};
	DevArray<int> spStraddle, spCount, spTarget, spSend, spRecv;
	std::vector<uint8_t> spOwners;
	bool spOwnersDirty = false;
	float spBounds[SHARD_MAX_RANKS + 1] = {0};
	b2hip_all_gather_fn gatherFn = nullptr;
	void* gatherUser = nullptr;
	int* spHost = nullptr;
	const int* spSendWiped = nullptr;
	int* spHdrHost = nullptr;
	int* spHdrDev = nullptr;
	int spHdrSeq = 0;
	int* spOwnHost = nullptr;
	int* spOwnDev = nullptr;
	size_t spOwnCapRows = 0;
	size_t spHostWords = 0;
	int spPairCap = 2048, spToiBodyCap = 256, spToiProxyCap = 512;
	int spOwned[SHARD_MAX_RANKS] = {0}, spOwnedProxies[SHARD_MAX_RANKS] = {0};
	long long spMigratedTotal = 0, spResolves = 0, spPairsSent = 0;
	size_t spBytesStep = 0;
	int spContactsBeforeToi = 0, spToiOrderBefore = 0, spTailCap = 64;
	int spToiUnsafe = 0;
	bool spToiSettled = false;
	DevArray<int4> spTailKey;
	DevArray<int2> spVirt;
	bool spTapeRecord = false;
	std::vector<std::pair<int*, size_t> > spTape;
	b2hip_world* spTapeFrom = nullptr;
	size_t spTapeCursor = 0;
	long long spToiRedos = 0;
	size_t spUp = 0;
	DevArray<int> scanFlags;
	ScanFlags scanCtx;
	DevArray<unsigned> radixCounts, radixGroups;
	DevArray<int> radixGlobalHist;
	RadixStatus radixCtx;
	bool sortOnepass = true;
	long long statSorts = 0, statSortsOnepass = 0;
	DevArray<float> stateOut;
	DevArray<int> gridBar;
	int dfEpoch;
	bool noSideStream, profileDetail;
	int collideStage = -1;
	int solidRoundsEnv = 0;
	int collideSplitEnv = -1;
	bool collideUniOff = false;
	int collideSortEnv = -1;
	hipStream_t stream2 = nullptr;
	hipEvent_t evFork = nullptr, evJoin = nullptr;
	DevArray<int> consts;
	DevArray<unsigned long long> filterPairs;
	std::vector<int> nonStatic;
	bool orderDirty = false;
	DevArray<int> b_order, orderBody;
	DevArray<int> bigRoots;
	std::vector<int2> editOps;
	std::vector<int> proxyEdits;
	std::vector<int> fatEdits;
	bool proxyListsStale = false;
	DevArray<int2> d_editOps;
	b2hip_should_collide_fn filterFn = nullptr;
	void* filterUser = nullptr;
	bool refilterPending = false;
	b2hip_pre_solve_fn preSolveFn = nullptr;
	b2hip_pre_solve_batch_fn preSolveBatchFn = nullptr;
	b2hip_should_collide_batch_fn filterBatchFn = nullptr;
	void* preSolveUser = nullptr;
	bool postSolveOn = false;
	std::vector<b2hip_contact_impulse> postSolve;
	DevArray<float4> pre_o0, pre_o1, pre_oimp;
	DevArray<int4> pre_o3;
	DevArray<PreSolveRec> preRecs;
	DevArray<PostSolveRec> postRecs;
	DevArray<int> filterList, hostList;
	DevArray<int> b_adoptStage;
	DevArray<int> b_blk1, b_adopt, blkRows, blkRowStart, blkCursor, blkBodyStart, blkBodies, rowColor, blkBodyCount, blkBodyCursor;
	DevArray<float4> b_cutv;
	int blocksMaxWG = 0;
	int sweepMaxWG[3] = { 0, 0, 0 };
	int hubWaves = 8;
	bool sweepEnd = true;
	bool sweepTail = true;
	int tailRowsMax = 1024;
	int freshColors = 0;
	bool freshColorsPending = false;
	bool forceOnDevice = true;
	int rowMarks = 1;
	bool rowsWentEarly = false;
	bool sweepStamps = false;
	bool bodyWarm = true;
	bool restFlow = true;
	bool noHubBuild = false;
	bool noHubOrder = false;
	bool hubOrderAll = false;
	bool recoverOn = true;
	int* h_solverWord = nullptr;
	int* d_solverWord = nullptr;
	int solverSeq = 0;
	int colorRecoveries = 0;
	int solverRecoveries = 0;
	int sweepRowsMax = 60000;
	int restHub = 2;
	int restHubMaxWG = 0;
	int restMaxWG = 0;
	int restArrived = 0;
	int restRowsMax = 65536;
	long long launchCount = 0;
	long long familyLaunchesAtStart = 0; int familyLaunches = 0;
	int largeHintSteps = 120;
	int serialOrphansNext = 0;
	int adoptSticky = 0;
	bool adoptPasses = false;
	bool traceLaunches = false;
	bool tracePartition = false;
	bool traceRecovery = false;
	bool toiWhy = false;
	bool handoverWhy = false;
	bool shardTrace = false;
	double stepDeadlineS = 300.0;
	int pollDelayUs = 0;
	bool gridHalf = false;
	bool gridForced = false;
	int pairsLargeSticky = 0;
	int toiPreSolveReruns = 0;
	int toiGridRetries = 0;
	int toiChainContacts = 0;
	int recolorCountdown = 0;
	bool blocksTooBig = false;
// ... 330 lines not shown

static int ktBracket(b2hip_world* w, int mode, int kind)
{
	if (w->kernelTiming != mode) return 0;
	w->ktKind = kind;
	return ktRecord(w);
}

static int gridFor(size_t n, int block = 256, int maxBlocks = 2048)
{
	size_t g = (n + block - 1) / block;
	if (g < 1) g = 1;
	if (g > (size_t)maxBlocks) g = maxBlocks;
	return (int)g;
}

static int readState(b2hip_world* w)
{
	HIP_TRY(hipMemcpyAsync(w->h_dstate, w->d_state.p, sizeof(DState), hipMemcpyDeviceToHost, w->stream));
	HIP_TRY(hipStreamSynchronize(w->stream));
	return 0;
}

static int pollPublished(b2hip_world* w, volatile const int* seq, int want, const char* what)
{
	bool drained = false;
	std::chrono::steady_clock::time_point drainedAt;
	const auto startedAt = std::chrono::steady_clock::now();
	for (unsigned spins = 1; *seq != want; ++spins)
	{
		if ((spins & 0x3fff) == 0)
		{
			const hipError_t q = hipStreamQuery(w->stream);
			if (q != hipSuccess && q != hipErrorNotReady) return setError(B2HIP_ERR_HIP, std::string(what) + ": " + hipGetErrorString(q));
			if (q == hipSuccess)
			{
				const auto now = std::chrono::steady_clock::now();
				if (!drained) { drained = true; drainedAt = now; }
				else if (now - drainedAt > std::chrono::seconds(2)) return setError(B2HIP_ERR_HIP, std::string(what) + " was not published (the stream has drained)");
			}
			else drained = false;
			if (std::chrono::duration<double>(std::chrono::steady_clock::now() - startedAt).count() > w->stepDeadlineS)
				return setError(B2HIP_ERR_HIP, std::string(what) + ": the device did not finish the step within the deadline (B2HIP_STEP_DEADLINE_S)");
		}
#if defined(__x86_64__)
		__builtin_ia32_pause();
#endif
	}
	std::atomic_thread_fence(std::memory_order_acquire);
	return 0;
}

static int awaitColors(b2hip_world* w)
{
	if (int rc = pollPublished(w, (volatile const int*)&w->h_pub2->pubSeq, w->pubSeq2, "colour state")) return rc;
	memcpy(w->h_dstate, w->h_pub2, offsetof(DState, pubSeq));
	return 0;
}

static int awaitCensus(b2hip_world* w)
{
	if (w->pollDelayUs > 0) std::this_thread::sleep_for(std::chrono::microseconds(w->pollDelayUs));
	if (int rc = pollPublished(w, (volatile const int*)&w->h_pub->pubSeq, w->pubSeq, "island census")) return rc;
	memcpy(w->h_dstate, w->h_pub, offsetof(DState, pubSeq));
	return 0;
}

static bool envSet(const char* k) { return getenv(k) != nullptr; }
static bool envOn(const char* k) { const char* e = getenv(k); return e && atoi(e); }
static int envInt(const char* k, int unset) { const char* e = getenv(k); return e ? atoi(e) : unset; }

static void readSwitches(b2hip_world* w)
{
	DW& d = w->dw;
	w->debugSync = envSet("B2HIP_DEBUG");
	w->traceLaunches = envSet("B2HIP_TRACE_LAUNCHES");
	w->debugTrace = envSet("B2HIP_TRACE");
	w->forceLarge = envInt("B2HIP_FORCE_LARGE", 0);
	w->kernelTimingLaunches = envSet("B2HIP_SOLVER_LAUNCHES");
	w->noSideStream = envSet("B2HIP_NO_SIDE_STREAM");
	w->profileDetail = envInt("B2HIP_PROFILE_DETAIL", 1) != 0;
	if (const char* e = getenv("B2HIP_SOLID_ROUNDS")) { const int v = atoi(e); w->solidRoundsEnv = (v == 1 || v == 2 || v == 4 || v == 8) ? v : 0; }
	w->collideSplitEnv = envInt("B2HIP_COLLIDE_SPLIT", -1);
	w->collideUniOff = envInt("B2HIP_COLLIDE_UNI", 1) == 0;
	w->collideSortEnv = envInt("B2HIP_COLLIDE_SORT", -1);
	w->sortOnepass = envInt("B2HIP_SORT_ONEPASS", 1) != 0;
	d.keysetKeep = envInt("B2HIP_KEYSET_KEEP", 1) != 0 ? 1 : 0;
	d.keysetMaxFill = std::min(std::max(envInt("B2HIP_KEYSET_MAX_FILL", 37), 1), 90);
	w->collideStage = envInt("B2HIP_COLLIDE_STAGE", -1);
	w->noSweepBlocks = envSet("B2HIP_NO_SWEEP_BLOCKS");
	w->tracePartition = envSet("B2HIP_TRACE_PARTITION");
	w->traceRecovery = envSet("B2HIP_TRACE_RECOVERY");
	if (const char* e = getenv("B2HIP_GRID_HALF")) { w->gridForced = true; w->gridHalf = atoi(e) != 0; d.gridHalf = w->gridHalf ? 1 : 0; }
	d.noChainCreate = envSet("B2HIP_TOI_NO_CHAIN_CREATE") ? 1 : 0;
	d.noOwnIdBlocks = envSet("B2HIP_NO_OWN_ID_BLOCKS") ? 1 : envSet("B2HIP_OWN_ID_BLOCKS_ALL") ? -1 : 0;
	w->noBlocks = envSet("B2HIP_NO_BLOCKS");
	w->blockLanes = 0;
	if (const char* e = getenv("B2HIP_BLOCK_LANES")) w->blockLanes = atoi(e) == 512 ? 512 : (atoi(e) == 256 ? 256 : (atoi(e) == 1024 ? 1024 : 0));
	w->toiSerialOnly = envSet("B2HIP_TOI_SERIAL");
	w->toiSyncOnly = envSet("B2HIP_TOI_SYNC");
	w->toiDomWideOnly = envSet("B2HIP_TOI_DOM_WIDE");
	w->noToiSpecDomains = envSet("B2HIP_TOI_NO_SPEC_DOMAINS");
	w->debugAssumeFreshGrid = envSet("B2HIP_DEBUG_ASSUME_FRESH_GRID");
	w->toiNoDomains = envSet("B2HIP_TOI_NO_DOMAINS");
	w->toiWhy = envSet("B2HIP_TOI_WHY");
	w->handoverWhy = envSet("B2HIP_HANDOVER_WHY");
	w->shardTrace = envOn("B2HIP_SHARD_TRACE");
	w->recoverOn = !envOn("B2HIP_NO_RECOVER");
	w->noCensusPoll = envOn("B2HIP_NO_CENSUS_POLL");
	w->noStatePoll = envOn("B2HIP_NO_STATE_POLL");
	w->lazyReadback = envOn("B2HIP_LAZY_READBACK");
	w->earlyRowsMin = envInt("B2HIP_EARLY_ROWS_MIN", w->earlyRowsMin);
	w->stepDeadlineS = getenv("B2HIP_STEP_DEADLINE_S") ? atof(getenv("B2HIP_STEP_DEADLINE_S")) : 300.0;
	w->pollDelayUs = envInt("B2HIP_TEST_POLL_DELAY_US", 0);
	d.bigChunks = envSet("B2HIP_BIG_CHUNKS") ? 1 : 0;
	d.smallMaxW = TINY_ISLAND_MAX_W;
	if (const char* e = getenv("B2HIP_SMALL_MAX_W")) d.smallMaxW = std::max(1, std::min((int)SMALL_ISLAND_MAX_W, atoi(e)));
	d.noFreeBodies = envOn("B2HIP_NO_FREE_BODIES") ? 1 : 0;
	d.testMaxColors = envInt("B2HIP_TEST_MAX_COLORS", 0);
	d.testColorRounds = envInt("B2HIP_TEST_COLOR_ROUNDS", 0);
	d.testSpinMax = std::max(0, envInt("B2HIP_TEST_SPIN_MAX", 0));
	d.restPoll = getenv("B2HIP_REST_POLL") ? std::max(1, std::min(16, atoi(getenv("B2HIP_REST_POLL")))) : 1;
	d.hubSerial = envOn("B2HIP_HUB_SERIAL") ? 1 : 0;
	w->hubWaves = envInt("B2HIP_HUB_WAVES", 0) == 1 ? 1 : 8;
	w->sweepEnd = !envOn("B2HIP_NO_SWEEP_END") && !envSet("B2HIP_HUB_WAVES");
	w->sweepTail = w->sweepEnd && !envOn("B2HIP_NO_TAIL");
	w->sweepStamps = envSet("B2HIP_SWEEP_STAMPS");
	w->rowMarks = envOn("B2HIP_ROW_MARKS_CHECK") ? 2 : envOn("B2HIP_NO_ROW_MARKS") ? 0 : 1;
	w->bodyWarm = !envOn("B2HIP_NO_BODY_WARM");
	w->restFlow = w->sweepEnd && !envOn("B2HIP_NO_REST");
	w->noHubBuild = envOn("B2HIP_NO_HUB_BUILD");
	w->noHubOrder = envOn("B2HIP_NO_HUB_ORDER");
	w->hubOrderAll = envOn("B2HIP_HUB_ORDER");
	if (getenv("B2HIP_SWEEP_ROWS_MAX")) w->sweepRowsMax = std::max(1, atoi(getenv("B2HIP_SWEEP_ROWS_MAX")));
	w->restHub = getenv("B2HIP_REST_HUB") ? std::max(0, std::min(2, atoi(getenv("B2HIP_REST_HUB")))) : 2;
	w->restRowsMax = getenv("B2HIP_REST_ROWS") ? std::min(atoi(getenv("B2HIP_REST_ROWS")), REST_ROWS_MAX - COLOR_SMALL_MAX) : 65536;
	w->tailRowsMax = envInt("B2HIP_TAIL_ROWS", SWEEP_END_LANES);
	d.hubWide = (w->sweepEnd && !d.hubSerial && envInt("B2HIP_HUB_WIDE", 1) != 0) ? 1 : 0;
}

static int ensureCapacity(b2hip_world* w, size_t needContacts)
{
	hipStream_t s = w->stream;
	const size_t nb = std::max<size_t>(w->bodies.size(), 1);
	const size_t np = std::max<size_t>(w->fixtures.size(), 1);
	int rc = 0;
#define ENS(arr, n) do { rc = w->arr.ensure((n), s); if (rc) return rc; } while (0)
	ENS(d_state, 1);
	ENS(b_pos, nb); ENS(b_pos0, nb); ENS(b_vel, nb); ENS(b_xf, nb); ENS(b_mass, nb); ENS(b_damp, nb); ENS(b_force, nb);
	ENS(b_flags, nb); ENS(b_wake, nb); ENS(b_rowDirty, nb); ENS(b_order, nb); ENS(orderBody, nb); ENS(bigRoots, SHARD_BIG_MAX);
	ENS(p_fat, np); ENS(p_body, np); ENS(p_shape, np); ENS(p_key, np); ENS(p_filter0, np); ENS(p_filter1, np); ENS(p_mat, np);
	ENS(b_proxyHead, nb); ENS(p_next, np);
	ENS(d_shapes, std::max<size_t>(w->shapes.size(), 1));
	ENS(d_joints, std::max<size_t>(w->joints.size(), 1));
	ENS(d_gears, std::max<size_t>(w->gears.size(), 1));
	ENS(solveSnapJoints, w->recoverOn ? std::max<size_t>(w->joints.size(), 1) : 1); ENS(solveSnapGears, w->recoverOn ? std::max<size_t>(w->gears.size(), 1) : 1);
	ENS(jadjStart, nb + 2); ENS(jadj, 2 * w->joints.size() + 2); ENS(rootJointStart, nb + 2); ENS(rootJointCursor, nb);
	ENS(lj_list, w->joints.size() + 2); ENS(rootJointOkay, nb);
	const size_t capPairs = std::max<size_t>(std::max<size_t>(8 * np + 4096, w->pairKey.cap), w->pairCapHint);
	const size_t capContacts = std::max<size_t>(needContacts + capPairs, 1024);
	for (int k = 0; k < 2; ++k)
	{
		ENS(c_ids[k], capContacts); ENS(c_key[k], capContacts); ENS(c_flags[k], capContacts); ENS(c_mat[k], capContacts);
		ENS(c_man0[k], capContacts); ENS(c_man1[k], capContacts); ENS(c_imp[k], capContacts); ENS(c_man3[k], capContacts);
		ENS(c_color[k], capContacts); ENS(c_mgr[k], capContacts);
	}
	const size_t cc = w->c_ids[0].cap;
	{
		size_t want = (size_t)nextPow2(2 * cc);
		if (w->ht_keys.cap < want)
		{
			const bool had = w->ht_keys.cap != 0;
			rc = w->ht_keys.ensure(want, s, false);
			if (rc) return rc;
			static const int one = 1;
			if (had) HIP_TRY(hipMemcpyAsync(&w->d_state.p->c.ksStale, &one, sizeof(int), hipMemcpyHostToDevice, s));
		}
	}
	ENS(parent, nb); ENS(rootSeed, nb); ENS(rootBodies, nb); ENS(rootContacts, nb); ENS(rootJoints, nb); ENS(rootIsland, nb);
	ENS(deg, nb + 1); ENS(adjStart, nb + 2); ENS(adjCursor, nb); ENS(adj, 2 * cc); ENS(adjSlot, cc);
	ENS(rootScanIn, nb + 1); ENS(rootScanOut, nb + 2);
	ENS(si_root, nb + 1); ENS(si_bodyStart, nb + 2); ENS(si_contactStart, nb + 2); ENS(si_wStart, nb + 2); ENS(si_maxLevel, nb + 1);
	ENS(si_bodies, nb); ENS(si_contacts, cc); ENS(si_level, cc); ENS(si_stack, nb); ENS(si_lastLevel, nb);
	ENS(b_slot, nb); ENS(b_island, nb); ENS(chunkFirst, (nb + cc) / (TINY_CHUNK_LANES / 2) + 4);
	ENS(li_bodies, nb); ENS(li_contacts, cc); ENS(li_roots, nb); ENS(li_color, cc);
	ENS(colorCount, cc + 2 + COLOR_SLOT_PADDED * COLOR_SLOT_STRIDE); ENS(colorStart, cc + 2); ENS(colorCursor, cc + 2 + COLOR_SLOT_PADDED * COLOR_SLOT_STRIDE); ENS(li_sorted, cc); ENS(li_ref, cc);
	ENS(bodyClaim, nb); ENS(bodyColorMask, nb); ENS(bodyActive, nb); ENS(bodyRest, nb); ENS(b_posv, nb); ENS(evKey, cc); ENS(evInfo, cc); ENS(uncolList, COLOR_SMALL_MAX); ENS(compactList, COLOR_SMALL_MAX); ENS(hubRowOf, cc); ENS(hubList, cc); ENS(hubDelta, cc); ENS(hubMeta, 8); ENS(hubFirst, nb); ENS(solveSnapBody, w->recoverOn ? 6 * nb : 1); ENS(solveSnapImp, w->recoverOn ? cc : 1); ENS(solveSnapCFlags, w->recoverOn ? cc : 1); ENS(rootPen, ROOT_PEN_SLOTS * nb); ENS(rootDone, nb); ENS(rootSleepMin, nb);
	if (w->lc.cap < (size_t)LC_WORDS * cc)
	{
		rc = w->lc.ensure((size_t)LC_WORDS * cc, s, false, false);
		if (rc) return rc;
	}
	if (w->warmDelta.cap < 4 * cc)
	{
		rc = w->warmDelta.ensure(4 * cc, s, false, false);
		if (rc) return rc;
	}
	ENS(moveBuf, 2 * np + 64);
	const size_t gridSize = (size_t)nextPow2(2 * np);
	ENS(gridCount, gridSize); ENS(gridStart, gridSize + 2); ENS(gridCursor, gridSize); ENS(gridItems, np); ENS(gridFat, np); ENS(arriveTree, (size_t)ARRIVE_SITES * TREE_WORDS); ENS(largeProxies, np); ENS(largeMoves, 2 * np + 64);
	ENS(pairKey, capPairs); ENS(pairKey2, capPairs); ENS(pairProxy, capPairs); ENS(pairProxy2, capPairs);
	ENS(pairFirst, capPairs + 1); ENS(pairRank, capPairs + 2);
	const size_t maxScanN = std::max(std::max(nb + 2, gridSize + 2), std::max(cc + 2, capPairs + 2));
	const size_t radixTiles = capPairs / RADIX_TILE + 2;
	ENS(radixHist, RADIX_DIGITS * radixTiles + 2); ENS(radixHistScan, RADIX_DIGITS * radixTiles + 4);
	ENS(scanTmp, 3 * (std::max(maxScanN, RADIX_DIGITS * radixTiles) / SCAN_TILE + 8));
	ENS(scanTmp4, 3 * (maxScanN / SCAN_TILE + 8));
	ENS(scanFlags, std::max(maxScanN, RADIX_DIGITS * radixTiles) / SCAN_TILE + 8);
	const size_t onepassTiles = w->sortOnepass ? std::min<size_t>(radixTiles, RADIX_ONEPASS_MAX_TILES) : 0;
	if (onepassTiles)
	{
		rc = w->radixCounts.ensure(onepassTiles * RADIX_DIGITS, s, false); if (rc) return rc;
		rc = w->radixGroups.ensure((onepassTiles / RADIX_GROUP + 1) * RADIX_DIGITS, s, false); if (rc) return rc;
		ENS(radixGlobalHist, 2 * RADIX_MAX_PASSES * RADIX_DIGITS);
	}
	ENS(keepFlag, cc + 1); ENS(keepScan, cc + 2);
	ENS(toiList, cc); ENS(toiPos2c, cc); ENS(toiDestroyList, cc); ENS(toiNewList, TOI_NEW_LIST_MAX);
	ENS(b_toiGroup, nb); ENS(toiGroups, nb); ENS(toiGroupCount, std::min<size_t>(nb, TOI_GROUPS_MAX)); ENS(toiGroupList, std::min<size_t>(nb, TOI_GROUPS_MAX) * CHAIN_ADJ_MAX); ENS(toiMoved, TOI_MOVED_ALL_MAX); ENS(toiNew, 8 * TOI_NEWPAIR_MAX); ENS(toiParent, nb); ENS(toiDomOf, nb); ENS(toiDomRoot, TOI_DOMAINS_MAX); ENS(toiDomCount, TOI_DOMAINS_MAX); ENS(toiDomBase, TOI_DOMAINS_MAX); ENS(toiDomFill, TOI_DOMAINS_MAX); ENS(toiDomFailed, TOI_DOMAINS_MAX); ENS(toiDomEvents, TOI_DOMAINS_MAX); ENS(toiDomList, cc); ENS(toiHull, np); ENS(snapBody, 5 * nb); ENS(snapFat, np);
	{
		const size_t nPre = hasPreSolve(w) ? cc : 1, nPost = w->postSolveOn ? cc : 1, nFil = hasFilter(w) ? cc : 1;
		ENS(pre_o0, nPre); ENS(pre_o1, nPre); ENS(pre_oimp, nPre); ENS(pre_o3, nPre); ENS(preRecs, nPre);
		ENS(postRecs, nPost); ENS(filterList, nFil);
		ENS(toiLog, listenerOn(w) && w->def.continuous ? cc : 1);
		ENS(toiVerdict, hasPreSolve(w) && w->def.continuous ? cc : 1);
		ENS(hostList, std::max<size_t>(std::max(4 * nPre, nFil), hasFilter(w) ? capPairs : 1));
	}
	ENS(b_blk1, nb); ENS(b_adopt, nb); ENS(b_adoptStage, 3 * nb); ENS(blkRows, (size_t)(MAX_BLOCKS + 2) * BLK_SLOT); ENS(blkRowStart, MAX_BLOCKS + 2); ENS(blkCursor, (size_t)(MAX_BLOCKS + 2) * BLK_SLOT); ENS(blkBodyCount, (size_t)(MAX_BLOCKS + 2) * BLK_SLOT); ENS(blkBodyCursor, (size_t)(MAX_BLOCKS + 2) * BLK_SLOT);
	ENS(blkBodyStart, MAX_BLOCKS + 2); ENS(blkBodies, nb); ENS(rowColor, cc); ENS(b_cutv, nb);
	ENS(b_owner, w->spatial ? nb : 1); ENS(spNewOwner, w->spatial ? nb : 1); ENS(spAwake, w->spatial ? nb : 1); ENS(spStraddle, w->spatial ? std::max<size_t>(w->spStraddle.cap, 4096) : 1);
	ENS(spCount, w->spatial ? (size_t)SP_RESOLVE_MAX * SHARD_MAX_RANKS : 1); ENS(spTarget, w->spatial ? SP_RESOLVE_MAX : 1);
	ENS(spTailKey, w->spatial ? capContacts : 1); ENS(spVirt, w->spatial ? SP_TAIL_MAX + 1 : 1);
	ENS(stateOut, 12 * nb + sizeof(DState) / sizeof(float) + 4);
	ENS(consts, 16);
	ENS(gridBar, 32);
#undef ENS
	w->scanCtx.words = w->scanFlags.p;
	w->scanCtx.count = w->scanFlags.cap;
	w->scanCtx.abortWord = &w->d_state.p->c.overflow;
	w->radixCtx.counts = w->radixCounts.p; w->radixCtx.countsCap = w->radixCounts.cap;
	w->radixCtx.groups = w->radixGroups.p; w->radixCtx.groupsCap = w->radixGroups.cap;
	w->radixCtx.hist = w->radixGlobalHist.p;
	w->radixCtx.maxTiles = w->sortOnepass ? (int)std::min<size_t>(std::min<size_t>(w->radixCounts.cap / RADIX_DIGITS, (w->radixGroups.cap / RADIX_DIGITS) * RADIX_GROUP), RADIX_ONEPASS_MAX_TILES) : 0;
	w->radixCtx.abortWord = &w->d_state.p->c.overflow;
	if (w->h_stateCap < 12 * nb + sizeof(DState) / sizeof(float) + 4)
	{
		ensureRows(w);
		float* old = w->h_state;
		w->h_state = nullptr;
		w->h_stateCap = 12 * nb * 2 + sizeof(DState) / sizeof(float) + 4;
		HIP_TRY(hipHostMalloc((void**)&w->h_state, w->h_stateCap * sizeof(float), hipHostMallocMapped | hipHostMallocCoherent));
		HIP_TRY(hipHostGetDevicePointer((void**)&w->d_hstate, w->h_state, 0));
		if (old)
		{
			memcpy(w->h_state, old, w->stateCount * 10 * sizeof(float));
			(void)hipHostFree(old);
		}
	}

	DW& d = w->dw;
	d.st = w->d_state.p;
	d.nBodies = (int)w->bodies.size();
	d.nProxies = (int)w->fixtures.size();
	d.nJoints = (int)w->joints.size();
	d.nShapes = (int)w->shapes.size();
	d.capContacts = (int)cc;
	d.capPairs = (int)w->pairKey.cap;
	d.capMoves = (int)w->moveBuf.cap;
	d.htMask = (uint32_t)(w->ht_keys.cap - 1);
	d.gridMask = (uint32_t)(gridSize - 1);
	d.b_pos = w->b_pos.p; d.b_pos0 = w->b_pos0.p; d.b_vel = w->b_vel.p; d.b_xf = w->b_xf.p; d.b_mass = w->b_mass.p;
	d.b_damp = w->b_damp.p; d.b_force = w->b_force.p; d.b_flags = w->b_flags.p; d.b_wake = w->b_wake.p; d.b_rowDirty = w->b_rowDirty.p;
	d.b_order = w->b_order.p; d.orderBody = w->orderBody.p; d.bigRoots = w->bigRoots.p;
	d.p_fat = w->p_fat.p; d.p_body = w->p_body.p; d.p_shape = w->p_shape.p; d.p_key = w->p_key.p;
	d.p_filter0 = w->p_filter0.p; d.p_filter1 = w->p_filter1.p; d.p_mat = w->p_mat.p; d.shapes = w->d_shapes.p;
	for (int k = 0; k < 2; ++k)
	{
		d.ca[k].ids = w->c_ids[k].p; d.ca[k].key = w->c_key[k].p; d.ca[k].flags = w->c_flags[k].p; d.ca[k].mat = w->c_mat[k].p;
		d.ca[k].man0 = w->c_man0[k].p; d.ca[k].man1 = w->c_man1[k].p; d.ca[k].imp = w->c_imp[k].p; d.ca[k].man3 = w->c_man3[k].p;
		d.ca[k].color = w->c_color[k].p; d.ca[k].mgr = w->c_mgr[k].p;
	}
	d.ht_keys = w->ht_keys.p;
	d.joints = w->d_joints.p; d.solveSnapJoints = w->solveSnapJoints.p; d.solveSnapGears = w->solveSnapGears.p; d.solveSnapBody = w->solveSnapBody.p; d.solveSnapImp = w->solveSnapImp.p; d.solveSnapCFlags = w->solveSnapCFlags.p;
	d.gears = w->d_gears.p;
	d.jadjStart = w->jadjStart.p; d.jadj = w->jadj.p; d.rootJointStart = w->rootJointStart.p;
	d.rootJointCursor = w->rootJointCursor.p; d.lj_list = w->lj_list.p; d.rootJointOkay = w->rootJointOkay.p;
	d.parent = w->parent.p; d.rootSeed = w->rootSeed.p; d.rootBodies = w->rootBodies.p; d.rootContacts = w->rootContacts.p;
	d.rootJoints = w->rootJoints.p; d.rootScanIn = w->rootScanIn.p; d.rootScanOut = w->rootScanOut.p; d.rootIsland = w->rootIsland.p;
	d.deg = w->deg.p; d.adjStart = w->adjStart.p; d.adjCursor = w->adjCursor.p; d.adj = w->adj.p; d.adjSlot = w->adjSlot.p;
	d.si_root = w->si_root.p; d.si_bodyStart = w->si_bodyStart.p; d.si_contactStart = w->si_contactStart.p; d.si_wStart = w->si_wStart.p;
	d.si_maxLevel = w->si_maxLevel.p; d.si_bodies = w->si_bodies.p; d.si_contacts = w->si_contacts.p; d.si_level = w->si_level.p;
	d.si_stack = w->si_stack.p; d.si_lastLevel = w->si_lastLevel.p; d.b_slot = w->b_slot.p; d.b_island = w->b_island.p;
	d.chunkFirst = w->chunkFirst.p;
	d.li_bodies = w->li_bodies.p; d.li_contacts = w->li_contacts.p; d.li_roots = w->li_roots.p; d.li_color = w->li_color.p;
	d.colorCount = w->colorCount.p; d.colorStart = w->colorStart.p; d.colorCursor = w->colorCursor.p; d.li_sorted = w->li_sorted.p; d.li_ref = w->li_ref.p;
	d.bodyClaim = w->bodyClaim.p; d.bodyColorMask = w->bodyColorMask.p; d.bodyActive = w->bodyActive.p; d.bodyRest = w->bodyRest.p; d.b_posv = w->b_posv.p; d.dfRank = nullptr; d.dfInbox = nullptr; d.evKey = w->evKey.p; d.evInfo = w->evInfo.p; d.eventsOn = w->eventsOn ? 1 : 0; d.uncolList = w->uncolList.p; d.compactList = w->compactList.p; d.hubRowOf = w->hubRowOf.p; d.hubList = w->hubList.p; d.hubDelta = w->hubDelta.p; d.hubMeta = w->hubMeta.p; d.hubFirst = w->hubFirst.p; d.lc = w->lc.p; d.warmDelta = w->warmDelta.p; d.rootPen = w->rootPen.p;
	d.rootDone = w->rootDone.p; d.rootSleepMin = w->rootSleepMin.p;
	d.moveBuf = w->moveBuf.p; d.gridCount = w->gridCount.p; d.gridStart = w->gridStart.p; d.gridCursor = w->gridCursor.p;
	d.gridItems = w->gridItems.p; d.gridFat = w->gridFat.p; d.arriveTree = w->arriveTree.p; d.largeProxies = w->largeProxies.p; d.largeMoves = w->largeMoves.p;
	d.pairKey = w->pairKey.p; d.pairProxy = w->pairProxy.p; d.pairKey2 = w->pairKey2.p; d.pairProxy2 = w->pairProxy2.p;
// ... 271 lines not shown
			const float2 mat = make_float2(f.friction, f.restitution);
			HIP_TRY(hipMemcpy(w->p_mat.p + id, &mat, sizeof(float2), hipMemcpyHostToDevice));
		}
		w->proxyEdits.clear();
		w->fatEdits.clear();
	}

	if (!w->pendingMoves.empty())
	{
		rc = readState(w);
		if (rc) return rc;
		int have = w->h_dstate->c.nMoves;
		HIP_TRY(hipMemcpyAsync(w->moveBuf.p + have, w->pendingMoves.data(), w->pendingMoves.size() * sizeof(int), hipMemcpyHostToDevice, s));
		int total = have + (int)w->pendingMoves.size();
		HIP_TRY(hipMemcpyAsync(&w->d_state.p->c.nMoves, &total, sizeof(int), hipMemcpyHostToDevice, s));
		HIP_TRY(hipStreamSynchronize(s));
		w->pendingMoves.clear();
	}
	const int consts[3] = { (int)w->bodies.size(), (int)(w->dw.gridMask + 1), (int)w->bodies.size() + 1 };
	if (consts[0] != w->constsUploaded[0] || consts[1] != w->constsUploaded[1] || w->consts.p != w->constsUploadedAt)
	{
		HIP_TRY(hipMemcpyAsync(w->consts.p, consts, sizeof(int) * 2, hipMemcpyHostToDevice, s));
		HIP_TRY(hipMemcpyAsync(w->consts.p + 4, &consts[2], sizeof(int), hipMemcpyHostToDevice, s));
		HIP_TRY(hipStreamSynchronize(s));
		w->constsUploaded[0] = consts[0];
		w->constsUploaded[1] = consts[1];
		w->constsUploadedAt = w->consts.p;
	}
	return 0;
}

static int applyPendingFilters(b2hip_world* w)
{
	if (w->pendingFilter.empty()) return 0;
	std::vector<unsigned long long> keys(w->pendingFilter.size());
	for (size_t k = 0; k < keys.size(); ++k)
	{
		const unsigned a = (unsigned)std::min(w->pendingFilter[k].first, w->pendingFilter[k].second);
		const unsigned b = (unsigned)std::max(w->pendingFilter[k].first, w->pendingFilter[k].second);
		keys[k] = ((unsigned long long)a << 32) | b;
	}
	std::sort(keys.begin(), keys.end());
	keys.erase(std::unique(keys.begin(), keys.end()), keys.end());
	int rc = w->filterPairs.ensure(keys.size(), w->stream, false, false);
	if (rc) return rc;
	HIP_TRY(hipMemcpyAsync(w->filterPairs.p, keys.data(), keys.size() * sizeof(unsigned long long), hipMemcpyHostToDevice, w->stream));
	LAUNCH(w, k_flag_filter, gridFor(w->dw.capContacts), 256, w->dw, w->filterPairs.p, (int)keys.size());
	HIP_TRY(hipStreamSynchronize(w->stream));
	w->pendingFilter.clear();
	w->refilterPending = true;
	return 0;
}

static int downloadState(b2hip_world* w, int clearForces, bool skipRowsIfRedo = false);
static int startEarlyRows(b2hip_world* w);

static int applyEditOps(b2hip_world* w, bool betweenSteps)
{
	if (w->editOps.empty()) return 0;
	bool destroys = false;
	for (size_t k = 0; k < w->editOps.size(); ++k) destroys = destroys || w->editOps[k].x == EDIT_DESTROY_BODY || w->editOps[k].x == EDIT_DESTROY_FIXTURE;
	int rc = w->d_editOps.ensure(w->editOps.size(), w->stream, false, false);
	if (rc) return rc;
	HIP_TRY(hipMemcpyAsync(w->d_editOps.p, w->editOps.data(), w->editOps.size() * sizeof(int2), hipMemcpyHostToDevice, w->stream));
	DW& d = w->dw;
	LAUNCH(w, k_apply_edits, 1, 1024, d, (const int2*)w->d_editOps.p, (int)w->editOps.size());
	if (destroys)
	{
		LAUNCH(w, k_edit_keepflags, gridFor(d.capContacts), 256, d);
		deviceExclusiveScan<int>(w->stream, d.keepFlag, d.keepScan, d.scanTmp, w->scanCtx, &d.st->c.nContacts, d.capContacts);
		LAUNCH(w, k_compact_contacts, gridFor(d.capContacts), 256, d);
		LAUNCH(w, k_edit_finish, 1, 1, d);
		if (betweenSteps)
		{
			rc = downloadState(w, 0);
			if (rc) return rc;
			w->stateCount = w->bodies.size();
			++w->mirrorEpoch;
		}
	}
	rc = readState(w);
	if (rc) return rc;
	w->editOps.clear();
	w->lastContacts = w->h_dstate->c.nContacts;
	w->last.nContacts = w->lastContacts;
	return 0;
}
```

Before: 362.4.

## Fuse contact compaction into collide kernel via decoupled look-back scan

Result: faster. 371.5 (median of 6 runs) (+2.5%).

```diff
diff --git a/box2d-mt_amd/csrc/b2d_kernels_collide.h b/box2d-mt_amd/csrc/b2d_kernels_collide.h
--- a/box2d-mt_amd/csrc/b2d_kernels_collide.h
+++ b/box2d-mt_amd/csrc/b2d_kernels_collide.h
@@ -3,6 +3,7 @@
 
 #include "b2d_world.h"
 #include "b2d_toi.h"
+#include "b2d_scan.h"
 
 __device__ __forceinline__ Xf loadXf(const float4* b_xf, int body)
 {
@@ -205,316 +206,62 @@
 		__float_as_uint(a.z) == __float_as_uint(b.z) && __float_as_uint(a.w) == __float_as_uint(b.w);
 }
 
+struct DW;
+__device__ __forceinline__ bool keysetMaintained(const DW& W);
+__device__ __forceinline__ bool htDelete(const DW& W, uint32_t mask, uint64_t key);
+
+struct CollideCompactArgs
+{
+	unsigned* counts;
+	unsigned* groups;
+	int* abortWord;
+	unsigned tag;
+	int chunk;
+};
+template <bool ON> struct CollideManifold
+{
+	__device__ __forceinline__ void set(float4, float4, float4) {}
+	__device__ __forceinline__ void set3(int4) {}
+	__device__ __forceinline__ float4 man0() const { return make_float4(0, 0, 0, 0); }
+	__device__ __forceinline__ float4 man1() const { return make_float4(0, 0, 0, 0); }
+	__device__ __forceinline__ float4 imp() const { return make_float4(0, 0, 0, 0); }
+	__device__ __forceinline__ int4 man3() const { return make_int4(0, 0, 0, 0); }
+};
+template <> struct CollideManifold<true>
+{
+	float4 m0, m1, mi;
+	int4 m3;
+	__device__ __forceinline__ void set(float4 a, float4 b, float4 c) { m0 = a; m1 = b; mi = c; }
+	__device__ __forceinline__ void set3(int4 a) { m3 = a; }
+	__device__ __forceinline__ float4 man0() const { return m0; }
+	__device__ __forceinline__ float4 man1() const { return m1; }
+	__device__ __forceinline__ float4 imp() const { return mi; }
+	__device__ __forceinline__ int4 man3() const { return m3; }
+};
+#define COLLIDE_GROUP 64
+__device__ __forceinline__ const unsigned* lookBackWord(const CollideCompactArgs& cc, int chunkId, int q)
+{
+	const int inGroup = chunkId % COLLIDE_GROUP;
+	return q < inGroup ? cc.counts + (chunkId - inGroup) + q : cc.groups + (q - inGroup);
+}
+
 template <int STAGE, bool ORDER = true>
 __global__ __launch_bounds__(256) void
 __attribute__((amdgpu_waves_per_eu((!ORDER && !STAGE) ? 4 : 1, (!ORDER && !STAGE) ? 4 : 8)))
 k_collide(DW W, int sortTile)
 {
-	b2dPhaseStamp(W);
-	DState* S = W.st;
-	const int n = S->c.nContacts;
-	const ContactArrays& C = W.ca[S->cur];
-	int nDestroy = 0, nTouch = 0;
-	__shared__ int s_bin[64];
-	__shared__ int s_perm[256];
-	__shared__ __attribute__((aligned(16))) unsigned char s_raw[STAGE ? ((512 * sizeof(ShapeRec) > TOI_ORDER_SCRATCH_BYTES || !ORDER) ? 512 * sizeof(ShapeRec) : TOI_ORDER_SCRATCH_BYTES) : (ORDER ? TOI_ORDER_SCRATCH_BYTES : 16)];
-	ShapeRec* const s_shape = (ShapeRec*)s_raw;
-	__shared__ __attribute__((aligned(16))) ShapeRec s_uni[2];
-	__shared__ int s_uniId[2];
-	const bool uniOn = !STAGE && (sortTile & 4) != 0;
-	sortTile &= 3;
-	if (uniOn)
-	{
-		const int i0 = (int)(blockIdx.x * blockDim.x);
-		int idA = 0, idB = 0;
-		if (i0 < n)
-		{
-			const int4 ids0 = C.ids[i0];
-			idA = W.p_shape[ids0.x];
-			idB = W.p_shape[ids0.y];
-		}
-		static_assert(sizeof(ShapeRec) % 4 == 0, "ShapeRec is copied word by word");
-		constexpr int RW = (int)(sizeof(ShapeRec) / 4);
-		if (threadIdx.x < 2 * RW)
-		{
-			const int which = (int)threadIdx.x / RW, word = (int)threadIdx.x % RW;
-			((uint32_t*)&s_uni[which])[word] = ((const uint32_t*)(W.shapes + (which ? idB : idA)))[word];
-		}
-		if (threadIdx.x == 0) { s_uniId[0] = idA; s_uniId[1] = idB; }
-		__syncthreads();
-	}
-	for (int base = blockIdx.x * blockDim.x; base < n; base += gridDim.x * blockDim.x)
-	{
-		int i = base + (int)threadIdx.x;
-		if (sortTile)
-		{
-			const int key = i < n ? collideClassKey(W, C, i) : 63;
-			if (threadIdx.x < 64) s_bin[threadIdx.x] = 0;
-			__syncthreads();
-			const int within = atomicAdd(&s_bin[key], 1);
-			__syncthreads();
-			if (threadIdx.x < 64)
-			{
-				const int v = s_bin[threadIdx.x];
-				int incl = v;
-				for (int off = 1; off < 64; off <<= 1)
-				{
-					const int o = __shfl_up(incl, off);
-					if ((int)threadIdx.x >= off) incl += o;
-				}
-				s_bin[threadIdx.x] = incl - v;
-			}
-			__syncthreads();
-			s_perm[s_bin[key] + within] = (int)threadIdx.x;
-			__syncthreads();
-			i = base + s_perm[threadIdx.x];
-		}
-		if (i >= n) continue;
-		int4 ids = C.ids[i];
-		uint32_t flags = C.flags[i];
-		if (flags & CF_FOREIGN)
-		{
-			int keepF = 1;
-			if (flags & CF_FILTER)
-			{
-				const bool ok = bodiesShouldCollide(W, ids.w, ids.z) &&
-					filterShouldCollide(W.p_filter0[ids.x], W.p_filter1[ids.x], W.p_filter0[ids.y], W.p_filter1[ids.y]);
-				if (!ok) keepF = 0; else flags &= ~CF_FILTER;
-			}
-			if (keepF && (bodyActiveForContact(W.b_flags[ids.z]) || bodyActiveForContact(W.b_flags[ids.w])))
-			{
-				const float4 fA = W.p_fat[ids.x], fB = W.p_fat[ids.y];
-				AABB boxA, boxB;
-				boxA.lo = v2(fA.x, fA.y); boxA.hi = v2(fA.z, fA.w);
-				boxB.lo = v2(fB.x, fB.y); boxB.hi = v2(fB.z, fB.w);
-				if (!b2dAabbOverlap(boxA, boxB)) keepF = 0;
-			}
-			if (!keepF)
-			{
-				flags |= CF_DESTROY;
-				++nDestroy;
-				if (flags & CF_TOI_CANDIDATE) b2dStoreAgentI(&W.toiDestroyList[atomicAdd(&S->c.nToiDestroy, 1)], i);
-			}
-			C.flags[i] = flags;
-			W.keepFlag[i] = keepF;
-			continue;
-		}
-		const int4 m3 = C.man3[i];
-		const float4 oldImp = C.imp[i];
-		const float4 o0 = C.man0[i], o1 = C.man1[i];
-		const int proxyA = ids.x, proxyB = ids.y, bodyA = ids.z, bodyB = ids.w;
-		uint32_t bfA = W.b_flags[bodyA], bfB = W.b_flags[bodyB];
-		const float4 fatA = W.p_fat[proxyA], fatB = W.p_fat[proxyB];
-		const int shapeA = W.p_shape[proxyA], shapeB = W.p_shape[proxyB];
-		const Xf xfA = loadXf(W.b_xf, bodyA), xfB = loadXf(W.b_xf, bodyB);
-		int keep = 1;
-
-		if (flags & CF_FILTER)
-		{
-			bool ok = bodiesShouldCollide(W, bodyB, bodyA) &&
-				(W.userFilter ? (flags & CF_USER_REJECT) == 0
-				              : filterShouldCollide(W.p_filter0[proxyA], W.p_filter1[proxyA], W.p_filter0[proxyB], W.p_filter1[proxyB]));
-			flags &= ~CF_USER_REJECT;
-			if (!ok)
-			{
-				keep = 0;
-			}
-			else
-			{
-				flags &= ~CF_FILTER;
-			}
-		}
-
-		flags &= ~(CF_PRESOLVE | CF_VC_ONE_POINT);
-		bool active = bodyActiveForContact(bfA) || bodyActiveForContact(bfB);
-		if (keep && active)
-		{
-			AABB boxA, boxB;
-			boxA.lo = v2(fatA.x, fatA.y); boxA.hi = v2(fatA.z, fatA.w);
-			boxB.lo = v2(fatB.x, fatB.y); boxB.hi = v2(fatB.z, fatB.w);
-			bool overlap = b2dAabbOverlap(boxA, boxB);
-			if (!overlap)
-			{
-				keep = 0;
-			}
-			else if (flags & CF_FOREIGN)
-			{
-			}
-			else
-			{
-				const uint32_t oldId0 = (uint32_t)m3.x, oldId1 = (uint32_t)m3.y;
-				const int oldCount = m3.w;
-				flags |= CF_ENABLED;
-				bool wasTouching = (flags & CF_TOUCHING) != 0;
-				bool touching = false;
-				bool sensor = (flags & CF_SENSOR) != 0;
-				float4 o0s = make_float4(0, 0, 0, 0), o1s = o0s;
-				Manifold mf;
-				mf.pointCount = 0;
-				mf.type = m3.z;
-				mf.id[0] = oldId0;
-				mf.id[1] = oldId1;
-				if (sensor)
-				{
-					const GjkProxy pA = b2dProxy(W.shapes + shapeA);
-					const GjkProxy pB = b2dProxy(W.shapes + shapeB);
-					GjkCache cache;
-					cache.count = 0;
-					cache.metric = 0.0f;
-					for (int k = 0; k < 3; ++k) cache.indexA[k] = cache.indexB[k] = 0;
-					GjkOutput dist;
-					b2dDistance(dist, cache, pA, xfA, pB, xfB, true);
-					touching = dist.distance < 10.0f * B2D_EPSILON;
-					mf.pointCount = 0;
-				}
-				else
-				{
-					const ShapeRec* sA = W.shapes + shapeA;
-					const ShapeRec* sB = W.shapes + shapeB;
-					if (STAGE)
-					{
-						static_assert(sizeof(ShapeRec) % 8 == 0, "ShapeRec is copied in 8-byte pieces");
-						const float2* gA = (const float2*)sA;
-						const float2* gB = (const float2*)sB;
-						float2* lA = (float2*)&s_shape[2 * threadIdx.x];
-						float2* lB = (float2*)&s_shape[2 * threadIdx.x + 1];
-#pragma unroll
-						for (int q = 0; q < (int)(sizeof(ShapeRec) / 8); ++q) { lA[q] = gA[q]; lB[q] = gB[q]; }
-						sA = &s_shape[2 * threadIdx.x];
-						sB = &s_shape[2 * threadIdx.x + 1];
-					}
-					o0s = o0;
-					o1s = o1;
-					mf.localNormal = v2(o0.x, o0.y);
-					mf.localPoint = v2(o0.z, o0.w);
-					mf.p[0] = v2(o1.x, o1.y);
-					mf.p[1] = v2(o1.z, o1.w);
-					mf.id[0] = oldId0;
-					mf.id[1] = oldId1;
-					bool evaluated = false;
-					if (uniOn)
-					{
-						const int u0 = s_uniId[0], u1 = s_uniId[1];
-						const bool a0 = shapeA == u0, b0 = shapeB == u0;
-						if ((a0 || shapeA == u1) && (b0 || shapeB == u1))
-						{
-							const ShapeRec* lA = &s_uni[a0 ? 0 : 1];
-							const ShapeRec* lB = &s_uni[b0 ? 0 : 1];
-							if (lA->type == B2D_SHAPE_POLYGON && lB->type == B2D_SHAPE_POLYGON && lA->count == 4 && lB->count == 4)
-							{
-								b2dCollidePolygons<4>(&mf, lA, xfA, lB, xfB);
-								evaluated = true;
-							}
-						}
-					}
-					if (!evaluated) b2dEvaluate(&mf, sA, xfA, sB, xfB);
-					touching = mf.pointCount > 0;
-					float ni[2], ti[2];
-					ni[0] = oldImp.x; ti[0] = oldImp.y; ni[1] = oldImp.z; ti[1] = oldImp.w;
-					for (int k = 0; k < mf.pointCount; ++k)
-					{
-						mf.ni[k] = 0.0f;
-						mf.ti[k] = 0.0f;
-						uint32_t id2 = mf.id[k];
-						if (oldCount > 0 && oldId0 == id2)
-						{
-							mf.ni[k] = oldImp.x;
-							mf.ti[k] = oldImp.y;
-						}
-						else if (oldCount > 1 && oldId1 == id2)
-						{
-							mf.ni[k] = oldImp.z;
-							mf.ti[k] = oldImp.w;
-						}
-						ni[k] = mf.ni[k];
-						ti[k] = mf.ti[k];
-					}
-					if (touching != wasTouching)
-					{
-						W.b_wake[bodyA] = 1;
-					}
-					{
-						const float4 n0 = make_float4(mf.localNormal.x, mf.localNormal.y, mf.localPoint.x, mf.localPoint.y);
-						const float4 n1 = make_float4(mf.p[0].x, mf.p[0].y, mf.p[1].x, mf.p[1].y);
-						const float4 nI = make_float4(ni[0], ti[0], ni[1], ti[1]);
-						if (!b2dSameBits4(n0, o0)) C.man0[i] = n0;
-						if (!b2dSameBits4(n1, o1)) C.man1[i] = n1;
-						if (!b2dSameBits4(nI, oldImp)) C.imp[i] = nI;
-					}
-				}
-				if (W.preSolveOn && !sensor && touching)
-				{
-					W.pre_o0[i] = o0s;
-					W.pre_o1[i] = o1s;
-					W.pre_oimp[i] = oldImp;
-					W.pre_o3[i] = m3;
-					flags |= CF_PRESOLVE;
-				}
-				{
-					const int4 n3 = make_int4((int)mf.id[0], (int)mf.id[1], mf.type, mf.pointCount);
-					if (n3.x != m3.x || n3.y != m3.y || n3.z != m3.z || n3.w != m3.w) C.man3[i] = n3;
-				}
-				if (touching) flags |= CF_TOUCHING; else flags &= ~CF_TOUCHING;
-			}
-		}
-
-		if (!keep)
-		{
-			if (W.eventsOn && (flags & CF_REPORTED))
-			{
-				const int e = atomicAdd(&S->c.nEvents, 1);
-				if (e < W.capContacts)
-				{
-					W.evKey[e] = C.key[i];
-					W.evInfo[e] = make_int4(proxyA, proxyB, 1, -1);
-				}
-			}
-			flags |= CF_DESTROY;
-			++nDestroy;
-			if (flags & CF_TOI_CANDIDATE) b2dStoreAgentI(&W.toiDestroyList[atomicAdd(&S->c.nToiDestroy, 1)], i);
-			int pc = C.man3[i].w;
-			if (pc > 0 && (flags & (CF_SENSOR | CF_FOREIGN)) == 0)
-			{
-				W.b_wake[bodyA] = 1;
-				W.b_wake[bodyB] = 1;
-			}
-		}
-		else if ((flags & (CF_TOUCHING | CF_FOREIGN)) == CF_TOUCHING)
-		{
-			++nTouch;
-		}
-		C.flags[i] = flags;
-		W.keepFlag[i] = keep;
-	}
-	{
-		__shared__ int s_census[2];
-		if (threadIdx.x == 0) { s_census[0] = 0; s_census[1] = 0; }
-		__syncthreads();
-		nDestroy = waveSumInt(nDestroy);
-		nTouch = waveSumInt(nTouch);
-		if (waveLane() == 0)
-		{
-			if (nDestroy) atomicAdd(&s_census[0], nDestroy);
-			if (nTouch) atomicAdd(&s_census[1], nTouch);
-		}
-		__syncthreads();
-		const bool fit = (unsigned)W.capContacts <= TREE_SUM_MAX;
-		if (!fit && threadIdx.x == 0)
-		{
-			if (s_census[0]) atomicAdd(&S->c.nDestroy, s_census[0]);
-			if (s_census[1]) atomicAdd(&S->c.nTouching, s_census[1]);
-		}
-		unsigned t0 = 0u, t1 = 0u;
-		if (b2dLastBlockArrive(W, ARRIVE_COLLIDE, fit ? (unsigned)s_census[0] : 0u, fit ? (unsigned)s_census[1] : 0u, &t0, &t1))
-		{
-			if (threadIdx.x == 0)
-			{
-				if (t0) atomicAdd(&S->c.nDestroy, (int)t0);
-				if (t1) atomicAdd(&S->c.nTouching, (int)t1);
-			}
-			if (ORDER) toiOrderDestroy(W, s_raw);
-		}
-	}
+	constexpr bool COMPACT = false;
+	const CollideCompactArgs cc = CollideCompactArgs();
+#include "b2d_kernels_collide_body.h"
+}
+
+template <int STAGE, bool ORDER, bool COMPACT>
+__global__ __launch_bounds__(256) void
+__attribute__((amdgpu_waves_per_eu(4, 4)))
+k_collide(DW W, int sortTile, CollideCompactArgs cc)
+{
+	static_assert(STAGE == 0 && !ORDER && COMPACT, "the form that stores the compacted array: k_collide<0, false, true>");
+#include "b2d_kernels_collide_body.h"
 }
 
 __global__ __launch_bounds__(256) void k_toi_order_destroy(DW W)
@@ -728,10 +475,6 @@
 	}
 }
 
-struct DW;
-__device__ __forceinline__ bool keysetMaintained(const DW& W);
-__device__ __forceinline__ bool htDelete(const DW& W, uint32_t mask, uint64_t key);
-
 __global__ __launch_bounds__(256) void k_compact_contacts(DW W)
 {
 	b2dPhaseStamp(W);
diff --git a/box2d-mt_amd/csrc/b2d_kernels_collide_body.h b/box2d-mt_amd/csrc/b2d_kernels_collide_body.h
--- /dev/null
+++ b/box2d-mt_amd/csrc/b2d_kernels_collide_body.h
@@ -0,0 +1,424 @@
+	b2dPhaseStamp(W);
+	DState* S = W.st;
+	const int n = S->c.nContacts;
+	const ContactArrays& C = W.ca[S->cur];
+	int nDestroy = 0, nTouch = 0;
+	const bool ksOn = COMPACT && keysetMaintained(W);
+	const uint32_t ksMask = COMPACT ? S->c.ksMask : 0u;
+	__shared__ int s_bin[64];
+	__shared__ int s_perm[256];
+	__shared__ __attribute__((aligned(16))) unsigned char s_raw[STAGE ? ((512 * sizeof(ShapeRec) > TOI_ORDER_SCRATCH_BYTES || !ORDER) ? 512 * sizeof(ShapeRec) : TOI_ORDER_SCRATCH_BYTES) : (ORDER ? TOI_ORDER_SCRATCH_BYTES : 16)];
+	ShapeRec* const s_shape = (ShapeRec*)s_raw;
+	__shared__ __attribute__((aligned(16))) ShapeRec s_uni[2];
+	__shared__ int s_uniId[2];
+	const bool uniOn = !STAGE && (sortTile & 4) != 0;
+	sortTile &= 3;
+	auto stageUni = [&]()
+	{
+		const int i0 = COMPACT ? (int)blockIdx.x * cc.chunk : (int)(blockIdx.x * blockDim.x);
+		int idA = 0, idB = 0;
+		if (i0 < n)
+		{
+			const int4 ids0 = C.ids[i0];
+			idA = W.p_shape[ids0.x];
+			idB = W.p_shape[ids0.y];
+		}
+		static_assert(sizeof(ShapeRec) % 4 == 0, "ShapeRec is copied word by word");
+		constexpr int RW = (int)(sizeof(ShapeRec) / 4);
+		if (threadIdx.x < 2 * RW)
+		{
+			const int which = (int)threadIdx.x / RW, word = (int)threadIdx.x % RW;
+			((uint32_t*)&s_uni[which])[word] = ((const uint32_t*)(W.shapes + (which ? idB : idA)))[word];
+		}
+		if (threadIdx.x == 0) { s_uniId[0] = idA; s_uniId[1] = idB; }
+	};
+	if (uniOn && !COMPACT)
+	{
+		stageUni();
+		__syncthreads();
+	}
+	for (int base = COMPACT ? blockIdx.x * cc.chunk : blockIdx.x * blockDim.x; COMPACT || base < n; base += gridDim.x * blockDim.x)
+	{
+		int i = base + (int)threadIdx.x;
+		const bool valid = !COMPACT || ((int)threadIdx.x < cc.chunk && i < n);
+		if (COMPACT && !valid) i = 0;
+		if (!COMPACT && sortTile)
+		{
+			const int key = i < n ? collideClassKey(W, C, i) : 63;
+			if (threadIdx.x < 64) s_bin[threadIdx.x] = 0;
+			__syncthreads();
+			const int within = atomicAdd(&s_bin[key], 1);
+			__syncthreads();
+			if (threadIdx.x < 64)
+			{
+				const int v = s_bin[threadIdx.x];
+				int incl = v;
+				for (int off = 1; off < 64; off <<= 1)
+				{
+					const int o = __shfl_up(incl, off);
+					if ((int)threadIdx.x >= off) incl += o;
+				}
+				s_bin[threadIdx.x] = incl - v;
+			}
+			__syncthreads();
+			s_perm[s_bin[key] + within] = (int)threadIdx.x;
+			__syncthreads();
+			i = base + s_perm[threadIdx.x];
+		}
+		if (!COMPACT && i >= n) continue;
+		int4 ids = C.ids[i];
+		uint32_t flags = C.flags[i];
+		if (COMPACT && !valid) { ids = make_int4(0, 0, 0, 0); flags = 0u; }
+		if (!COMPACT && (flags & CF_FOREIGN))
+		{
+			int keepF = 1;
+			if (flags & CF_FILTER)
+			{
+				const bool ok = bodiesShouldCollide(W, ids.w, ids.z) &&
+					filterShouldCollide(W.p_filter0[ids.x], W.p_filter1[ids.x], W.p_filter0[ids.y], W.p_filter1[ids.y]);
+				if (!ok) keepF = 0; else flags &= ~CF_FILTER;
+			}
+			if (keepF && (bodyActiveForContact(W.b_flags[ids.z]) || bodyActiveForContact(W.b_flags[ids.w])))
+			{
+				const float4 fA = W.p_fat[ids.x], fB = W.p_fat[ids.y];
+				AABB boxA, boxB;
+				boxA.lo = v2(fA.x, fA.y); boxA.hi = v2(fA.z, fA.w);
+				boxB.lo = v2(fB.x, fB.y); boxB.hi = v2(fB.z, fB.w);
+				if (!b2dAabbOverlap(boxA, boxB)) keepF = 0;
+			}
+			if (!keepF)
+			{
+				flags |= CF_DESTROY;
+				++nDestroy;
+				if (flags & CF_TOI_CANDIDATE) b2dStoreAgentI(&W.toiDestroyList[atomicAdd(&S->c.nToiDestroy, 1)], i);
+			}
+			C.flags[i] = flags;
+			W.keepFlag[i] = keepF;
+			continue;
+		}
+		const int4 m3 = C.man3[i];
+		const float4 oldImp = C.imp[i];
+		const float4 o0 = C.man0[i], o1 = C.man1[i];
+		const int proxyA = ids.x, proxyB = ids.y, bodyA = ids.z, bodyB = ids.w;
+		uint32_t bfA = W.b_flags[bodyA], bfB = W.b_flags[bodyB];
+		const float4 fatA = W.p_fat[proxyA], fatB = W.p_fat[proxyB];
+		const int shapeA = W.p_shape[proxyA], shapeB = W.p_shape[proxyB];
+		const Xf xfA = loadXf(W.b_xf, bodyA), xfB = loadXf(W.b_xf, bodyB);
+		int keep = 1;
+
+		if (flags & CF_FILTER)
+		{
+			bool ok = bodiesShouldCollide(W, bodyB, bodyA) &&
+				(W.userFilter ? (flags & CF_USER_REJECT) == 0
+				              : filterShouldCollide(W.p_filter0[proxyA], W.p_filter1[proxyA], W.p_filter0[proxyB], W.p_filter1[proxyB]));
+			flags &= ~CF_USER_REJECT;
+			if (!ok)
+			{
+				keep = 0;
+			}
+			else
+			{
+				flags &= ~CF_FILTER;
+			}
+		}
+
+		flags &= ~(CF_PRESOLVE | CF_VC_ONE_POINT);
+		bool active = bodyActiveForContact(bfA) || bodyActiveForContact(bfB);
+		CollideManifold<COMPACT> now;
+		now.set(o0, o1, oldImp);
+		now.set3(m3);
+		int rank = 0;
+		unsigned early = 0u;
+		if (COMPACT)
+		{
+			__shared__ int s_waveKeep[4];
+			int stays = valid ? keep : 0;
+			if (stays && active && (fatB.x - fatA.z > 0.0f || fatB.y - fatA.w > 0.0f || fatA.x - fatB.z > 0.0f || fatA.y - fatB.w > 0.0f)) stays = 0;
+			const unsigned long long kb = __ballot(stays != 0);
+			const int lane = (int)threadIdx.x & 63, wave = (int)threadIdx.x >> 6;
+			rank = __popcll(kb & ((1ull << lane) - 1ull));
+			if (lane == 0) s_waveKeep[wave] = __popcll(kb);
+			if (uniOn) stageUni();
+			__syncthreads();
+			int chunkKeep = 0;
+			for (int q = 0; q < 4; ++q)
+			{
+				const int c = s_waveKeep[q];
+				chunkKeep += c;
+				if (q < wave) rank += c;
+			}
+			const int chunkId = (int)blockIdx.x, inGroup = chunkId % COLLIDE_GROUP;
+			if (threadIdx.x == 0) __hip_atomic_store(cc.counts + chunkId, (cc.tag << 16) | (unsigned)chunkKeep, __ATOMIC_RELAXED, __HIP_MEMORY_SCOPE_AGENT);
+			if (inGroup == COLLIDE_GROUP - 1 && wave == 0)
+			{
+				bool gaveUp = false;
+				int v = 0;
+				if (lane < COLLIDE_GROUP - 1)
+				{
+					const unsigned* src = cc.counts + (chunkId - inGroup) + lane;
+					v = radixAwait(src, __hip_atomic_load(src, __ATOMIC_RELAXED, __HIP_MEMORY_SCOPE_AGENT), cc.tag, cc.abortWord, gaveUp);
+				}
+				v = waveSumInt(v);
+				if (lane == 0) __hip_atomic_store(cc.groups + chunkId / COLLIDE_GROUP, (cc.tag << 16) | (unsigned)(v + chunkKeep), __ATOMIC_RELAXED, __HIP_MEMORY_SCOPE_AGENT);
+			}
+			if ((int)threadIdx.x < inGroup + chunkId / COLLIDE_GROUP)
+				early = __hip_atomic_load(lookBackWord(cc, chunkId, (int)threadIdx.x), __ATOMIC_RELAXED, __HIP_MEMORY_SCOPE_AGENT);
+		}
+		if (keep && active && valid)
+		{
+			AABB boxA, boxB;
+			boxA.lo = v2(fatA.x, fatA.y); boxA.hi = v2(fatA.z, fatA.w);
+			boxB.lo = v2(fatB.x, fatB.y); boxB.hi = v2(fatB.z, fatB.w);
+			bool overlap = b2dAabbOverlap(boxA, boxB);
+			if (!overlap)
+			{
+				keep = 0;
+			}
+			else if (flags & CF_FOREIGN)
+			{
+			}
+			else
+			{
+				const uint32_t oldId0 = (uint32_t)m3.x, oldId1 = (uint32_t)m3.y;
+				const int oldCount = m3.w;
+				flags |= CF_ENABLED;
+				bool wasTouching = (flags & CF_TOUCHING) != 0;
+				bool touching = false;
+				bool sensor = (flags & CF_SENSOR) != 0;
+				float4 o0s = make_float4(0, 0, 0, 0), o1s = o0s;
+				Manifold mf;
+				mf.pointCount = 0;
+				mf.type = m3.z;
+				mf.id[0] = oldId0;
+				mf.id[1] = oldId1;
+				if (sensor)
+				{
+					const GjkProxy pA = b2dProxy(W.shapes + shapeA);
+					const GjkProxy pB = b2dProxy(W.shapes + shapeB);
+					GjkCache cache;
+					cache.count = 0;
+					cache.metric = 0.0f;
+					for (int k = 0; k < 3; ++k) cache.indexA[k] = cache.indexB[k] = 0;
+					GjkOutput dist;
+					b2dDistance(dist, cache, pA, xfA, pB, xfB, true);
+					touching = dist.distance < 10.0f * B2D_EPSILON;
+					mf.pointCount = 0;
+				}
+				else
+				{
+					const ShapeRec* sA = W.shapes + shapeA;
+					const ShapeRec* sB = W.shapes + shapeB;
+					if (STAGE)
+					{
+						static_assert(sizeof(ShapeRec) % 8 == 0, "ShapeRec is copied in 8-byte pieces");
+						const float2* gA = (const float2*)sA;
+						const float2* gB = (const float2*)sB;
+						float2* lA = (float2*)&s_shape[2 * threadIdx.x];
+						float2* lB = (float2*)&s_shape[2 * threadIdx.x + 1];
+#pragma unroll
+						for (int q = 0; q < (int)(sizeof(ShapeRec) / 8); ++q) { lA[q] = gA[q]; lB[q] = gB[q]; }
+						sA = &s_shape[2 * threadIdx.x];
+						sB = &s_shape[2 * threadIdx.x + 1];
+					}
+					o0s = o0;
+					o1s = o1;
+					mf.localNormal = v2(o0.x, o0.y);
+					mf.localPoint = v2(o0.z, o0.w);
+					mf.p[0] = v2(o1.x, o1.y);
+					mf.p[1] = v2(o1.z, o1.w);
+					mf.id[0] = oldId0;
+					mf.id[1] = oldId1;
+					bool evaluated = false;
+					if (uniOn)
+					{
+						const int u0 = s_uniId[0], u1 = s_uniId[1];
+						const bool a0 = shapeA == u0, b0 = shapeB == u0;
+						if ((a0 || shapeA == u1) && (b0 || shapeB == u1))
+						{
+							const ShapeRec* lA = &s_uni[a0 ? 0 : 1];
+							const ShapeRec* lB = &s_uni[b0 ? 0 : 1];
+							if (lA->type == B2D_SHAPE_POLYGON && lB->type == B2D_SHAPE_POLYGON && lA->count == 4 && lB->count == 4)
+							{
+								b2dCollidePolygons<4>(&mf, lA, xfA, lB, xfB);
+								evaluated = true;
+							}
+						}
+					}
+					if (!evaluated) b2dEvaluate(&mf, sA, xfA, sB, xfB);
+					touching = mf.pointCount > 0;
+					float ni[2], ti[2];
+					ni[0] = oldImp.x; ti[0] = oldImp.y; ni[1] = oldImp.z; ti[1] = oldImp.w;
+					for (int k = 0; k < mf.pointCount; ++k)
+					{
+						mf.ni[k] = 0.0f;
+						mf.ti[k] = 0.0f;
+						uint32_t id2 = mf.id[k];
+						if (oldCount > 0 && oldId0 == id2)
+						{
+							mf.ni[k] = oldImp.x;
+							mf.ti[k] = oldImp.y;
+						}
+						else if (oldCount > 1 && oldId1 == id2)
+						{
+							mf.ni[k] = oldImp.z;
+							mf.ti[k] = oldImp.w;
+						}
+						ni[k] = mf.ni[k];
+						ti[k] = mf.ti[k];
+					}
+					if (touching != wasTouching)
+					{
+						W.b_wake[bodyA] = 1;
+					}
+					{
+						const float4 n0 = make_float4(mf.localNormal.x, mf.localNormal.y, mf.localPoint.x, mf.localPoint.y);
+						const float4 n1 = make_float4(mf.p[0].x, mf.p[0].y, mf.p[1].x, mf.p[1].y);
+						const float4 nI = make_float4(ni[0], ti[0], ni[1], ti[1]);
+						if (COMPACT) now.set(n0, n1, nI);
+						else
+						{
+							if (!b2dSameBits4(n0, o0)) C.man0[i] = n0;
+							if (!b2dSameBits4(n1, o1)) C.man1[i] = n1;
+							if (!b2dSameBits4(nI, oldImp)) C.imp[i] = nI;
+						}
+					}
+				}
+				if (!COMPACT && W.preSolveOn && !sensor && touching)
+				{
+					W.pre_o0[i] = o0s;
+					W.pre_o1[i] = o1s;
+					W.pre_oimp[i] = oldImp;
+					W.pre_o3[i] = m3;
+					flags |= CF_PRESOLVE;
+				}
+				{
+					const int4 n3 = make_int4((int)mf.id[0], (int)mf.id[1], mf.type, mf.pointCount);
+					if (COMPACT) now.set3(n3);
+					else if (n3.x != m3.x || n3.y != m3.y || n3.z != m3.z || n3.w != m3.w) C.man3[i] = n3;
+				}
+				if (touching) flags |= CF_TOUCHING; else flags &= ~CF_TOUCHING;
+			}
+		}
+
+		if (COMPACT && !valid)
+		{
+		}
+		else if (!keep)
+		{
+			if (!COMPACT && W.eventsOn && (flags & CF_REPORTED))
+			{
+				const int e = atomicAdd(&S->c.nEvents, 1);
+				if (e < W.capContacts)
+				{
+					W.evKey[e] = C.key[i];
+					W.evInfo[e] = make_int4(proxyA, proxyB, 1, -1);
+				}
+			}
+			flags |= CF_DESTROY;
+			++nDestroy;
+			if (COMPACT)
+			{
+				if (flags & CF_TOI_CANDIDATE) atomicOr(cc.abortWord, SCAN_ABORT_BIT);
+			}
+			else if (flags & CF_TOI_CANDIDATE) b2dStoreAgentI(&W.toiDestroyList[atomicAdd(&S->c.nToiDestroy, 1)], i);
+			int pc = COMPACT ? m3.w : C.man3[i].w;
+			if (pc > 0 && (flags & (CF_SENSOR | CF_FOREIGN)) == 0)
+			{
+				W.b_wake[bodyA] = 1;
+				W.b_wake[bodyB] = 1;
+			}
+		}
+		else if ((flags & (CF_TOUCHING | CF_FOREIGN)) == CF_TOUCHING)
+		{
+			++nTouch;
+		}
+		if (!COMPACT)
+		{
+			C.flags[i] = flags;
+			W.keepFlag[i] = keep;
+		}
+		else
+		{
+			__shared__ int s_before[4];
+			const ContactArrays& B = W.ca[1 - S->cur];
+			const uint64_t key = C.key[i];
+			const float4 mat = C.mat[i];
+			const int color = C.color[i];
+			const int mgr = C.mgr[i];
+			const int chunkId = (int)blockIdx.x, group = chunkId / COLLIDE_GROUP, inGroup = chunkId % COLLIDE_GROUP;
+			int before = 0;
+			bool gaveUp = false;
+			for (int q = (int)threadIdx.x; q < inGroup + group; q += (int)blockDim.x)
+			{
+				const unsigned* src = lookBackWord(cc, chunkId, q);
+				before += radixAwait(src, q < (int)blockDim.x ? early : __hip_atomic_load(src, __ATOMIC_RELAXED, __HIP_MEMORY_SCOPE_AGENT), cc.tag, cc.abortWord, gaveUp);
+			}
+			before = waveSumInt(before);
+			if (waveLane() == 0) s_before[threadIdx.x >> 6] = before;
+			__syncthreads();
+			const int j = s_before[0] + s_before[1] + s_before[2] + s_before[3] + rank;
+			if (valid && keep && j <= i)
+			{
+				B.ids[j] = ids;
+				B.key[j] = key;
+				B.flags[j] = flags;
+				B.mat[j] = mat;
+				B.man0[j] = now.man0();
+				B.man1[j] = now.man1();
+				B.imp[j] = now.imp();
+				B.man3[j] = now.man3();
+				B.color[j] = color;
+				B.mgr[j] = mgr;
+				if (mgr >= 0) W.toiPos2c[mgr] = j;
+			}
+			else if (valid && !keep && ksOn)
+			{
+				if (!htDelete(W, ksMask, key + 1ull)) __hip_atomic_fetch_add(W.arriveTree + (size_t)ARRIVE_COMPACT * TREE_WORDS, 1ull, __ATOMIC_RELAXED, __HIP_MEMORY_SCOPE_AGENT);
+			}
+			break;
+		}
+	}
+	if (COMPACT)
+	{
+		if (blockIdx.x == 0 && threadIdx.x == 0 && (long long)n > (long long)gridDim.x * cc.chunk) atomicOr(cc.abortWord, SCAN_ABORT_BIT);
+	}
+	{
+		__shared__ int s_census[2];
+		if (threadIdx.x == 0) { s_census[0] = 0; s_census[1] = 0; }
+		__syncthreads();
+		nDestroy = waveSumInt(nDestroy);
+		nTouch = waveSumInt(nTouch);
+		if (waveLane() == 0)
+		{
+			if (nDestroy) atomicAdd(&s_census[0], nDestroy);
+			if (nTouch) atomicAdd(&s_census[1], nTouch);
+		}
+		__syncthreads();
+		const bool fit = (unsigned)W.capContacts <= TREE_SUM_MAX;
+		if (!fit && threadIdx.x == 0)
+		{
+			if (s_census[0]) atomicAdd(&S->c.nDestroy, s_census[0]);
+			if (s_census[1]) atomicAdd(&S->c.nTouching, s_census[1]);
+		}
+		unsigned t0 = 0u, t1 = 0u;
+		if (b2dLastBlockArrive(W, ARRIVE_COLLIDE, fit ? (unsigned)s_census[0] : 0u, fit ? (unsigned)s_census[1] : 0u, &t0, &t1))
+		{
+			if (threadIdx.x == 0)
+			{
+				if (t0) atomicAdd(&S->c.nDestroy, (int)t0);
+				if (t1) atomicAdd(&S->c.nTouching, (int)t1);
+				if (COMPACT)
+				{
+					S->c.nContacts = n - (int)t0;
+					S->cur = 1 - S->cur;
+					if (ksOn)
+					{
+						const unsigned long long lost = __hip_atomic_exchange(W.arriveTree + (size_t)ARRIVE_COMPACT * TREE_WORDS, 0ull, __ATOMIC_RELAXED, __HIP_MEMORY_SCOPE_AGENT);
+						S->c.ksStats[KS_TOMBSTONES] += (unsigned long long)t0 - lost;
+						if (lost) { S->c.ksStats[KS_NOT_FOUND] += lost; S->c.ksStale = 1; }
+					}
+				}
+			}
+			if (ORDER) toiOrderDestroy(W, s_raw);
+		}
+	}
diff --git a/box2d-mt_amd/csrc/b2hip_api_callbacks.h b/box2d-mt_amd/csrc/b2hip_api_callbacks.h
--- a/box2d-mt_amd/csrc/b2hip_api_callbacks.h
+++ b/box2d-mt_amd/csrc/b2hip_api_callbacks.h
@@ -227,6 +227,12 @@
 		stats[KS_STATS] = c.ksFill;
 		stats[KS_STATS + 1] = c.ksMask;
 		memcpy(out, stats + first, (size_t)count * sizeof(long long));
+		return 0;
+	}
+	case 24:
+	{
+		if (first != 0 || count != 1) return setError(B2HIP_ERR_INVALID, "narrow-phase statistics: [0, 1)");
+		memcpy(out, &w->statCollideCompact, sizeof(long long));
 		return 0;
 	}
 	default: return setError(B2HIP_ERR_INVALID, "bad array id");
diff --git a/box2d-mt_amd/csrc/b2hip_api_snapshot.h b/box2d-mt_amd/csrc/b2hip_api_snapshot.h
--- a/box2d-mt_amd/csrc/b2hip_api_snapshot.h
+++ b/box2d-mt_amd/csrc/b2hip_api_snapshot.h
@@ -303,6 +303,7 @@
 	w->shadowDev = nullptr;
 	w->stateCount = h.stateCount;
 	*w->h_dstate = ds;
+	w->contactsKnown = false;
 #define SNAP_UP(arr, s) do { if ((s).bytes && hipMemcpy(w->arr.p, (s).p, (s).bytes, hipMemcpyHostToDevice) != hipSuccess) return fail(setError(B2HIP_ERR_HIP, "snapshot upload failed (" #arr ")")); } while (0)
 	if (hipMemcpy(w->d_state.p, &ds, sizeof(DState), hipMemcpyHostToDevice) != hipSuccess) return fail(setError(B2HIP_ERR_HIP, "snapshot upload failed (state block)"));
 	w->pubSeq = ds.pubCount;
diff --git a/box2d-mt_amd/csrc/b2hip_api_step.h b/box2d-mt_amd/csrc/b2hip_api_step.h
--- a/box2d-mt_amd/csrc/b2hip_api_step.h
+++ b/box2d-mt_amd/csrc/b2hip_api_step.h
@@ -663,6 +663,7 @@
 		w->last.toiOverflow = c.toiOverflow;
 		if (c.toiOverflow) return setError(B2HIP_ERR_CAPACITY, "TOI event scratch overflow (flags " + std::to_string(c.toiOverflow) + ")");
 	}
+	w->contactsKnown = true;
 	if (w->sp.dt > 0.0f) w->inv_dt0 = w->sp.inv_dt;
 	if (w->def.continuous && w->sp.dt > 0.0f) w->stepComplete = c.toiIncomplete == 0;
 	w->stepActive = false;
diff --git a/box2d-mt_amd/csrc/b2hip_api_world.h b/box2d-mt_amd/csrc/b2hip_api_world.h
--- a/box2d-mt_amd/csrc/b2hip_api_world.h
+++ b/box2d-mt_amd/csrc/b2hip_api_world.h
@@ -208,7 +208,7 @@
 	w->li_bodies.release(); w->li_contacts.release(); w->li_roots.release(); w->li_color.release(); w->colorCount.release();
 	w->colorStart.release(); w->colorCursor.release(); w->li_sorted.release(); w->bodyClaim.release(); w->rootPen.release();
 	w->bodyActive.release(); w->bodyRest.release(); w->b_posv.release(); w->evKey.release(); w->evInfo.release(); w->uncolList.release(); w->compactList.release(); w->gridBar.release(); w->hubRowOf.release(); w->hubList.release(); w->hubDelta.release(); w->hubMeta.release(); w->hubFirst.release(); w->solveSnapBody.release(); w->solveSnapImp.release(); w->solveSnapCFlags.release(); w->solveSnapJoints.release(); w->solveSnapGears.release();
-	w->b_proxyHead.release(); w->p_next.release(); w->toiList.release(); w->toiPos2c.release(); w->toiDestroyList.release(); w->toiNewList.release();
+	w->b_proxyHead.release(); w->p_next.release(); w->toiList.release(); w->toiPos2c.release(); w->toiDestroyList.release(); w->toiNewList.release(); w->collideCounts.release(); w->collideGroups.release();
 	w->b_toiGroup.release(); w->toiGroups.release(); w->toiGroupCount.release(); w->toiGroupList.release(); w->toiMoved.release(); w->toiNew.release(); w->toiParent.release(); w->toiDomOf.release(); w->toiDomRoot.release(); w->toiDomCount.release(); w->toiDomBase.release(); w->toiDomFill.release(); w->toiDomFailed.release(); w->toiDomEvents.release(); w->toiDomList.release(); w->toiHull.release(); w->snapBody.release(); w->snapFat.release();
 	w->c_mgr[0].release(); w->c_mgr[1].release(); w->dbgPreVel.release(); w->dbgVel.release(); w->dbgLi.release();
 	w->rootSleepMin.release(); w->bodyColorMask.release(); w->rootDone.release(); w->lc.release(); w->warmDelta.release();
diff --git a/box2d-mt_amd/csrc/b2hip_host_phases.h b/box2d-mt_amd/csrc/b2hip_host_phases.h
--- a/box2d-mt_amd/csrc/b2hip_host_phases.h
+++ b/box2d-mt_amd/csrc/b2hip_host_phases.h
@@ -172,6 +172,7 @@
 
 static int findNewContacts(b2hip_world* w, bool sync)
 {
+	w->contactsKnown = false;
 	for (int attempt = 0; sync && attempt < 4; ++attempt)
 	{
 		int rc = findNewContactsOnce(w, true);
@@ -239,6 +240,36 @@
 	const bool stage = w->collideStage < 0 ? many : w->collideStage != 0;
 	const int sort = w->collideSortEnv < 0 ? (many ? 1 : 0) : (w->collideSortEnv != 0 ? 1 : 0);
 	const int uni = w->collideUniOff ? 0 : 4;
+	const bool known = w->contactsKnown;
+	w->contactsKnown = false;
+	bool compact = w->collideCompactOn && split && !stage && sort == 0 && known && w->h_dstate->c.nToiOrder == 0 && w->h_dstate->c.nContacts >= 0 &&
+		!d.preSolveOn && !d.eventsOn && !w->spatial && d.shardCount <= 1 && (unsigned)d.capContacts <= TREE_SUM_MAX;
+	if (compact)
+	{
+		hipStreamCaptureStatus capturing = hipStreamCaptureStatusNone;
+		(void)hipStreamIsCapturing(w->stream, &capturing);
+		compact = capturing == hipStreamCaptureStatusNone;
+	}
+	const size_t chunks = compact ? ((size_t)w->h_dstate->c.nContacts + w->collideChunk - 1) / w->collideChunk : 0;
+	if (compact && (chunks > w->collideCounts.cap || chunks / COLLIDE_GROUP + 1 > w->collideGroups.cap)) compact = false;
+	if (compact)
+	{
+		if (w->collideEpoch >= 0xffffu)
+		{
+			HIP_TRY(hipMemsetAsync(w->collideCounts.p, 0, w->collideCounts.cap * sizeof(unsigned), w->stream));
+			HIP_TRY(hipMemsetAsync(w->collideGroups.p, 0, w->collideGroups.cap * sizeof(unsigned), w->stream));
+			w->collideEpoch = 0u;
+		}
+		CollideCompactArgs cc;
+		cc.counts = w->collideCounts.p;
+		cc.groups = w->collideGroups.p;
+		cc.abortWord = w->scanCtx.abortWord;
+		cc.tag = ++w->collideEpoch;
+		cc.chunk = w->collideChunk;
+		w->statCollideCompact += 1;
+		LAUNCH(w, (k_collide<0, false, true>), (int)std::max<size_t>(chunks, 1), 256, d, uni, cc);
+		return ktBracket(w, 2, 5);
+	}
 	if (stage) LAUNCH(w, (k_collide<1, true>), gridFor(d.capContacts), 256, d, sort);
 	else if (split)
 	{
diff --git a/box2d-mt_amd/csrc/b2hip_host_world.h b/box2d-mt_amd/csrc/b2hip_host_world.h
--- a/box2d-mt_amd/csrc/b2hip_host_world.h
+++ b/box2d-mt_amd/csrc/b2hip_host_world.h
@@ -247,6 +247,12 @@
 	int collideStage = -1;
 	int solidRoundsEnv = 0;
 	int collideSplitEnv = -1;
+	bool collideCompactOn = true;
+	int collideChunk = 256;
+	bool contactsKnown = false;
+	DevArray<unsigned> collideCounts, collideGroups;
+	unsigned collideEpoch = 0;
+	long long statCollideCompact = 0;
 	bool collideUniOff = false;
 	int collideSortEnv = -1;
 	hipStream_t stream2 = nullptr;
@@ -743,6 +749,8 @@
 	w->profileDetail = envInt("B2HIP_PROFILE_DETAIL", 1) != 0;
 	if (const char* e = getenv("B2HIP_SOLID_ROUNDS")) { const int v = atoi(e); w->solidRoundsEnv = (v == 1 || v == 2 || v == 4 || v == 8) ? v : 0; }
 	w->collideSplitEnv = envInt("B2HIP_COLLIDE_SPLIT", -1);
+	w->collideCompactOn = envInt("B2HIP_COLLIDE_COMPACT", 1) != 0;
+	w->collideChunk = std::min(std::max(envInt("B2HIP_TEST_COLLIDE_CHUNK", 256), 1), 256);
 	w->collideUniOff = envInt("B2HIP_COLLIDE_UNI", 1) == 0;
 	w->collideSortEnv = envInt("B2HIP_COLLIDE_SORT", -1);
 	w->sortOnepass = envInt("B2HIP_SORT_ONEPASS", 1) != 0;
@@ -876,6 +884,12 @@
 		ENS(radixGlobalHist, 2 * RADIX_MAX_PASSES * RADIX_DIGITS);
 	}
 	ENS(keepFlag, cc + 1); ENS(keepScan, cc + 2);
+	if (w->collideCompactOn)
+	{
+		const size_t chunks = cc / (size_t)w->collideChunk + 2;
+		rc = w->collideCounts.ensure(chunks, s, false); if (rc) return rc;
+		rc = w->collideGroups.ensure(chunks / COLLIDE_GROUP + 2, s, false); if (rc) return rc;
+	}
 	ENS(toiList, cc); ENS(toiPos2c, cc); ENS(toiDestroyList, cc); ENS(toiNewList, TOI_NEW_LIST_MAX);
 	ENS(b_toiGroup, nb); ENS(toiGroups, nb); ENS(toiGroupCount, std::min<size_t>(nb, TOI_GROUPS_MAX)); ENS(toiGroupList, std::min<size_t>(nb, TOI_GROUPS_MAX) * CHAIN_ADJ_MAX); ENS(toiMoved, TOI_MOVED_ALL_MAX); ENS(toiNew, 8 * TOI_NEWPAIR_MAX); ENS(toiParent, nb); ENS(toiDomOf, nb); ENS(toiDomRoot, TOI_DOMAINS_MAX); ENS(toiDomCount, TOI_DOMAINS_MAX); ENS(toiDomBase, TOI_DOMAINS_MAX); ENS(toiDomFill, TOI_DOMAINS_MAX); ENS(toiDomFailed, TOI_DOMAINS_MAX); ENS(toiDomEvents, TOI_DOMAINS_MAX); ENS(toiDomList, cc); ENS(toiHull, np); ENS(snapBody, 5 * nb); ENS(snapFat, np);
 	{
@@ -1313,6 +1327,7 @@
 	rc = readState(w);
 	if (rc) return rc;
 	w->editOps.clear();
+	w->contactsKnown = true;
 	w->lastContacts = w->h_dstate->c.nContacts;
 	w->last.nContacts = w->lastContacts;
 	return 0;
```
